# peterarmstrong/corda

Measured on AMD Instinct MI355X. Metric: verified sigs/sec (whole node), Ed25519 + ECDSA-P256, at 1/2/4/8 MI355X, higher is better.
Workload: dtype u32

## Files before the change

corda_amd/csrc/cordagpu.cpp:

```cpp
#include <hip/hip_runtime.h>

#include <algorithm>
#include <atomic>
#include <chrono>
#include <cmath>
#include <cstdio>
#include <cstring>
#include <functional>
#include <initializer_list>
#include <memory>
#include <mutex>
#include <string>
#include <thread>
#include <vector>

#include "../../include/cordagpu.h"
#include "call_scope.h"
#include "engine.h"
#include "host_budget.h"
#include "host_pool.h"
#include "pool.h"
#include "rsa.h"
#include "table_budget.h"
#include "txsig_plan.h"

namespace cg24 {
const cgt::EngineVariant& variant();
}
namespace cg22 {
const cgt::EngineVariant& variant();
}

namespace {

thread_local std::string g_err;

int fail(int code, const char* fmt, const char* detail = "") {
  char buf[512];
  snprintf(buf, sizeof buf, fmt, detail);
  g_err = buf;
  return code;
}

int hip_fail(hipError_t e, const char* where) {
  char buf[512];
  snprintf(buf, sizeof buf, "%s: %s", where, hipGetErrorString(e));
  g_err = buf;
  return e == hipErrorOutOfMemory ? CG_ERR_NOMEM : CG_ERR_DEVICE;
}

#define HIP_TRY(expr, where)               \
  do {                                     \
    hipError_t _e = (expr);                \
    if (_e != hipSuccess) return hip_fail(_e, where); \
  } while (0)

bool env_flag(const char* name, bool dflt) {
  const char* v = getenv(name);
  return v ? (dflt ? v[0] != '0' : v[0] == '1') : dflt;
}
uint64_t env_u64(const char* name, uint64_t dflt) {
  const char* v = getenv(name);
  return v ? (uint64_t)strtoull(v, nullptr, 10) : dflt;
}

struct DevBuf {
  void* p = nullptr;
  size_t cap = 0;
  hipError_t ensure(size_t bytes) { return bytes <= cap ? hipSuccess : replace(bytes + bytes / 4 + 256); }
  hipError_t ensure_exact(size_t bytes) { return bytes <= cap ? hipSuccess : replace(bytes); }
  hipError_t replace(size_t want) {
    release();
    const hipError_t e = hipMalloc(&p, want);
    if (e == hipSuccess) cap = want;
    return e;
  }
  void release() {
    if (p) hipFree(p);
    p = nullptr;
    cap = 0;
  }
};

struct Need {
  DevBuf* buf;
  size_t bytes;
};
hipError_t ensure_all(std::initializer_list<Need> needs) {
  bool grow = false;
  for (const Need& n : needs) grow = grow || n.buf->cap < n.bytes;
  if (!grow) return hipSuccess;
  hipError_t e = hipDeviceSynchronize();
  for (const Need& n : needs)
    if (e == hipSuccess) e = n.buf->ensure(n.bytes);
  return e;
}

hipError_t stage(DevBuf& b, const void* src, size_t bytes, hipStream_t s, size_t room = 0) {
  hipError_t e = b.ensure(std::max<size_t>({bytes, room, 1}));
  if (e == hipSuccess && bytes) e = hipMemcpyAsync(b.p, src, bytes, hipMemcpyHostToDevice, s);
  return e;
}
size_t arena_room(uint64_t arena_len) { return ((arena_len + 3) & ~(uint64_t)3) + 16; }

struct HipStreams {
  using Stream = hipStream_t;
  using Event = hipEvent_t;
  using Error = hipError_t;
  static constexpr Error kOk = hipSuccess;
  Error record(Event e, Stream s) { return hipEventRecord(e, s); }
  Error wait(Stream s, Event e) { return hipStreamWaitEvent(s, e, 0); }
  Error sync(Stream s) { return hipStreamSynchronize(s); }
};

}

struct cg_ctx : cg::CallState<HipStreams> {
  int device = 0;
  uint64_t chunk = CG_DEFAULT_CHUNK_ITEMS;
  bool chunk_set = false;
  bool fault = false;
  cg::Fork fork = {{nullptr, nullptr, nullptr}, nullptr, {nullptr, nullptr, nullptr}, nullptr,
                   {nullptr, nullptr, nullptr}, nullptr};
  std::mutex mu;
  DevBuf keyprep, itemws, keys, items, arena, status, aux0, aux1, aux2;
  void* btab = nullptr;
  const cgt::EngineVariant* eng = nullptr;
  uint64_t tab_bytes = 0;
  DevBuf wide;
  bool rsa = false;
  DevBuf rsakeys, rsalist;
  uint32_t wide_max = cg::kKeyWideMax;
  DevBuf kcache;
  uint32_t wide_slots = 0;
  uint32_t wide_slots_max = cg::kKeyWideMax;
  uint32_t kc_bits = 32;
  bool kc_on = true;
  bool kc_dirty = true;
  bool kc_open = false;
  DevBuf txitems, msgs, tmpls, h_txs, h_comps, h_sigs, h_ids, h_txst;
  DevBuf sig12ws;
  DevBuf txvws, txvio;
  DevBuf ftxws;
  DevBuf bfws, bfin, bfio;
  DevBuf signers, signws;
  uint32_t n_signers = 0;
  DevBuf derivews;
  uint32_t derive_force = 0;
  DevBuf ec_signers, signecws;
  uint32_t n_ec_signers = 0;
  DevBuf rsa_signers, signrsaws;
  uint32_t n_rsa_signers = 0;
  hipStream_t copy2 = nullptr;
  cg::CountScratch count_scratch;
  std::unique_ptr<cg::HostPool> hpool;
  uint32_t host_req = 0;
  uint32_t quota = 1;
  bool counted = false;
  std::vector<hipEvent_t> seg;
  hipEvent_t tev[4] = {};
  std::vector<hipEvent_t> segt;
  std::vector<hipEvent_t> segtab;
  hipEvent_t backt[2] = {nullptr, nullptr};
  std::vector<hipEvent_t> fbt;
  std::vector<double> fbh;
  bool htrace = false;
  cg::StageTimer timer;
};

namespace {

std::atomic<unsigned> g_live_ctx{0};

const cgt::EngineVariant* const kVariants[] = {&cg::variant(), &cg24::variant(), &cg22::variant()};
constexpr int kNumVariants = 3;

std::vector<cgb::TableSet> table_sets() {
  std::vector<cgb::TableSet> v;
  for (const cgt::EngineVariant* e : kVariants) v.push_back({e->fixed_base_bits, (uint64_t)e->btab_bytes()});
  return v;
}

struct SharedTables {
  int device;
  int variant;
  void* p;
  unsigned refs;
};
std::mutex g_tab_mu;
std::vector<SharedTables> g_tabs;

hipError_t acquire_tables(int device, hipStream_t s, uint64_t budget, void** out, int* variant) {
  std::lock_guard<std::mutex> g(g_tab_mu);
  const std::vector<cgb::TableSet> sets = table_sets();
  int held = -1;
  for (const SharedTables& t : g_tabs)
    if (t.device == device && (held < 0 || t.variant < held)) held = t.variant;
  size_t free_b = 0, total_b = 0;
  if (hipMemGetInfo(&free_b, &total_b) != hipSuccess) free_b = 0;
  const int pick = cgb::pick_tables(sets.data(), kNumVariants, budget, free_b, held);
  if (pick < 0) return hipErrorInvalidValue;
  for (SharedTables& t : g_tabs)
    if (t.device == device && t.variant == pick) {
      ++t.refs;
      *out = t.p;
      *variant = pick;
      return hipSuccess;
    }
  hipError_t e = hipErrorOutOfMemory;
  for (int v = pick; v < kNumVariants; ++v) {
    if (budget && sets[v].bytes > budget) continue;
    void* p = nullptr;
    e = hipMalloc(&p, sets[v].bytes);
    if (e == hipSuccess) {
      DevBuf scratch;
      e = scratch.ensure(kVariants[v]->btab_scratch_bytes());
      if (e == hipSuccess) e = kVariants[v]->upload_constants();
      if (e == hipSuccess) e = kVariants[v]->init_btab(p, scratch.p, s);
      if (e == hipSuccess) e = hipStreamSynchronize(s);
      scratch.release();
      if (e == hipSuccess) {
        g_tabs.push_back({device, v, p, 1u});
        *out = p;
        *variant = v;
        return hipSuccess;
      }
      hipFree(p);
    }
    (void)hipGetLastError();
    if (e != hipErrorOutOfMemory || budget) break;
  }
  return e;
}

void release_tables(int device, void* p) {
  std::lock_guard<std::mutex> g(g_tab_mu);
  for (size_t i = 0; i < g_tabs.size(); ++i)
    if (g_tabs[i].device == device && g_tabs[i].p == p) {
      if (--g_tabs[i].refs == 0) {
        hipSetDevice(device);
        hipFree(p);
        g_tabs.erase(g_tabs.begin() + (ptrdiff_t)i);
      }
      return;
    }
}

unsigned host_threads_of(cg_ctx* c, uint64_t n) {
  if (n < (1u << 16)) return 1;
  const unsigned nt = cg::host_threads_for(c->host_req, cg::host_threads_env(), c->quota, g_live_ctx.load());
  if (nt <= 1) c->hpool.reset();
  else if (!c->hpool || c->hpool->threads() != nt) c->hpool.reset(new cg::HostPool(nt - 1));
  return nt;
}

void host_par(cg_ctx* c, uint64_t m, const std::function<void(uint64_t)>& fn) {
  if (m > 1 && c->hpool) {
    c->hpool->run(m, fn);
  } else {
    for (uint64_t t = 0; t < m; ++t) fn(t);
  }
}

HipStreams g_hip;
struct Call : cg::CallScope<HipStreams> {
  Call(cg_ctx* c, Form form) : CallScope(g_hip, *c, form) {}
  hipError_t open(void* hip_stream = nullptr) { return CallScope::open((hipStream_t)hip_stream); }
};

int enter(cg_ctx* c, const char* fn) {
  if (c->fault) return fail(CG_ERR_DEVICE, "%s: device fault (injected by cg_pool_inject_fault)", fn);
  HIP_TRY(hipSetDevice(c->device), "hipSetDevice");
  return CG_OK;
}

uint64_t chunk_of(const cg_ctx* c, uint64_t n) { return cg::equal_chunk(c->chunk, n); }

size_t item_half_bytes(const cg_ctx* c, uint64_t ws_items) { return (c->eng->item_ws_bytes(ws_items) + 255) & ~(size_t)255; }
hipError_t ensure_rsa(cg_ctx* c, uint32_t n_keys, uint64_t n_items) {
  if (!c->rsa) return hipSuccess;
  return ensure_all({{&c->rsakeys, cg::rsa_keys_bytes(n_keys)}, {&c->rsalist, cg::rsa_list_bytes(n_items)}});
}
hipError_t rsa_keyprep(cg_ctx* c, const cg::VerifyReq& r, hipStream_t s) {
  if (!c->rsa) return hipSuccess;
  return cg::launch_rsa_keyprep(r, c->rsakeys.p, s);
}
hipError_t rsa_items(cg_ctx* c, const cg::VerifyReq& r, hipStream_t s) {
  if (!c->rsa || r.n_items == 0) return hipSuccess;
  return cg::launch_rsa_items(r, c->rsakeys.p, c->rsalist.p, s);
}

hipError_t ensure_ws(cg_ctx* c, uint32_t n_keys, uint64_t ws_items, uint64_t call_items = 0) {
  {
// ... 698 lines not shown
  std::lock_guard<std::mutex> g(c->mu);
  if (const int rc = enter(c, "cg_sha256_batch_device")) return rc;
  Call call(c, Call::kDevice);
  HIP_TRY(call.open(hip_stream), "hipStreamWaitEvent");
  HIP_TRY(cg::launch_sha256(d_spans, n, d_arena, arena_len, d_digests, call.stream()), "launch_sha256");
  HIP_TRY(call.close(), "hipEventRecord");
  return CG_OK;
}

static int hash_batch(cg_ctx* c, const cg_span* spans, uint64_t n, const uint8_t* arena, uint64_t arena_len,
                      uint8_t* out, int which) {
  if (!c) return fail(CG_ERR_ARG, "hash batch: ctx is NULL");
  if (n && (!spans || !out)) return fail(CG_ERR_ARG, "hash batch: NULL buffer");
  if (n == 0) return CG_OK;
  const size_t dlen = which == 256 ? 32 : 64;
  std::lock_guard<std::mutex> g(c->mu);
  if (const int rc = enter(c, which == 256 ? "cg_sha256_batch" : "cg_sha512_batch")) return rc;
  hipStream_t s = c->stream;
  Call call(c, Call::kHost);
  HIP_TRY(call.open(), "hipStreamWaitEvent");
  HIP_TRY(stage(c->items, spans, sizeof(cg_span) * n, s), "H2D spans");
  HIP_TRY(stage(c->arena, arena, arena_len, s, arena_room(arena_len)), "H2D arena");
  HIP_TRY(c->aux0.ensure(dlen * n), "hipMalloc(digests)");
  HIP_TRY((which == 256 ? cg::launch_sha256 : cg::launch_sha512)((const cg_span*)c->items.p, n, (const uint8_t*)c->arena.p,
                                                                 arena_len, (uint8_t*)c->aux0.p, s), "launch_sha");
  HIP_TRY(hipMemcpyAsync(out, c->aux0.p, dlen * n, hipMemcpyDeviceToHost, s), "D2H digests");
  HIP_TRY(call.close(), "hipEventRecord");
  HIP_TRY(hipStreamSynchronize(s), "hipStreamSynchronize");
  return CG_OK;
}

int cg_sha256_batch(cg_ctx* c, const cg_span* spans, uint64_t n, const uint8_t* arena, uint64_t arena_len,
                    uint8_t* out) {
  return hash_batch(c, spans, n, arena, arena_len, out, 256);
}
int cg_sha512_batch(cg_ctx* c, const cg_span* spans, uint64_t n, const uint8_t* arena, uint64_t arena_len,
                    uint8_t* out) {
  return hash_batch(c, spans, n, arena, arena_len, out, 512);
}

int cg_tx_ids_device(cg_ctx* c, const cg_tx* d_txs, uint64_t n_tx, const cg_component* d_comps, uint64_t n_comps,
                     const uint8_t* d_arena, uint64_t arena_len, uint8_t* d_ids, uint8_t* d_status,
                     void* hip_stream) {
  if (!c) return fail(CG_ERR_ARG, "cg_tx_ids_device: ctx is NULL");
  std::lock_guard<std::mutex> g(c->mu);
  if (const int rc = enter(c, "cg_tx_ids_device")) return rc;
  HIP_TRY(ensure_all({{&c->aux2, cg::tx_ws_bytes(n_comps)}}), "hipMalloc(leaf ws)");
  Call call(c, Call::kDevice);
  HIP_TRY(call.open(hip_stream), "hipStreamWaitEvent");
  HIP_TRY(cg::launch_tx_ids(d_txs, n_tx, d_comps, n_comps, d_arena, arena_len, d_ids, d_status,
                            (uint8_t*)c->aux2.p, call.stream()), "launch_tx_ids");
  HIP_TRY(call.close(), "hipEventRecord");
  return CG_OK;
}

int cg_tx_ids(cg_ctx* c, const cg_tx* txs, uint64_t n_tx, const cg_component* comps, uint64_t n_comps,
              const uint8_t* arena, uint64_t arena_len, uint8_t* ids_out, uint8_t* status_out) {
  if (!c) return fail(CG_ERR_ARG, "cg_tx_ids: ctx is NULL");
  if (n_tx && (!txs || !ids_out || !status_out)) return fail(CG_ERR_ARG, "cg_tx_ids: NULL buffer");
  if (n_tx == 0) return CG_OK;
  std::lock_guard<std::mutex> g(c->mu);
  if (const int rc = enter(c, "cg_tx_ids")) return rc;
  hipStream_t s = c->stream;
  Call call(c, Call::kHost);
  HIP_TRY(call.open(), "hipStreamWaitEvent");
  HIP_TRY(stage(c->keys, txs, sizeof(cg_tx) * n_tx, s), "H2D txs");
  HIP_TRY(stage(c->items, comps, sizeof(cg_component) * n_comps, s), "H2D comps");
  HIP_TRY(stage(c->arena, arena, arena_len, s, arena_room(arena_len)), "H2D arena");
  HIP_TRY(c->aux0.ensure(32 * n_tx), "hipMalloc(ids)");
  HIP_TRY(c->status.ensure(n_tx), "hipMalloc(status)");
  HIP_TRY(c->aux2.ensure(cg::tx_ws_bytes(n_comps)), "hipMalloc(leaf ws)");
  HIP_TRY(cg::launch_tx_ids((const cg_tx*)c->keys.p, n_tx, (const cg_component*)c->items.p, n_comps,
                            (const uint8_t*)c->arena.p, arena_len, (uint8_t*)c->aux0.p, (uint8_t*)c->status.p,
                            (uint8_t*)c->aux2.p, s), "launch_tx_ids");
  HIP_TRY(hipMemcpyAsync(ids_out, c->aux0.p, 32 * n_tx, hipMemcpyDeviceToHost, s), "D2H ids");
  HIP_TRY(hipMemcpyAsync(status_out, c->status.p, n_tx, hipMemcpyDeviceToHost, s), "D2H status");
  HIP_TRY(call.close(), "hipEventRecord");
  HIP_TRY(hipStreamSynchronize(s), "hipStreamSynchronize");
  return CG_OK;
}

int cg_merkle_roots(cg_ctx* c, const uint8_t* leaves, const uint64_t* first, const uint32_t* count, uint64_t n,
                    uint8_t* roots_out, uint8_t* status_out) {
  if (!c) return fail(CG_ERR_ARG, "cg_merkle_roots: ctx is NULL");
  if (n && (!first || !count || !roots_out || !status_out)) return fail(CG_ERR_ARG, "cg_merkle_roots: NULL buffer");
  if (n == 0) return CG_OK;
  uint64_t total = 0, ws = 0;
  std::vector<uint64_t> wsoff(n);
  for (uint64_t j = 0; j < n; ++j) {
    if (first[j] + count[j] > total) total = first[j] + count[j];
    wsoff[j] = ws;
    ws += count[j];
  }
  std::lock_guard<std::mutex> g(c->mu);
  if (const int rc = enter(c, "cg_merkle_roots")) return rc;
  hipStream_t s = c->stream;
  Call call(c, Call::kHost);
  HIP_TRY(call.open(), "hipStreamWaitEvent");
  HIP_TRY(stage(c->arena, leaves, 32 * total, s), "H2D leaves");
  HIP_TRY(stage(c->keys, first, 8 * n, s), "H2D first");
  HIP_TRY(stage(c->items, count, 4 * n, s), "H2D count");
  HIP_TRY(stage(c->aux2, wsoff.data(), 8 * n, s), "H2D wsoff");
  HIP_TRY(c->aux0.ensure(32 * n), "hipMalloc(roots)");
  HIP_TRY(c->status.ensure(n), "hipMalloc(status)");
  HIP_TRY(c->aux1.ensure(32 * (ws ? ws : 1)), "hipMalloc(ws)");
  HIP_TRY(cg::launch_merkle_roots((const uint8_t*)c->arena.p, (const uint64_t*)c->keys.p, (const uint32_t*)c->items.p,
                                  n, (uint8_t*)c->aux0.p, (uint8_t*)c->status.p, (uint8_t*)c->aux1.p,
                                  (const uint64_t*)c->aux2.p, s),
          "launch_merkle_roots");
  HIP_TRY(hipMemcpyAsync(roots_out, c->aux0.p, 32 * n, hipMemcpyDeviceToHost, s), "D2H roots");
  HIP_TRY(hipMemcpyAsync(status_out, c->status.p, n, hipMemcpyDeviceToHost, s), "D2H status");
  HIP_TRY(call.close(), "hipEventRecord");
  HIP_TRY(hipStreamSynchronize(s), "hipStreamSynchronize");
  return CG_OK;
}

static uint64_t tmpl_slot(const cg_signable_tmpl* tmpls, uint32_t n_tmpls) {
  uint64_t maxlen = 0;
  for (uint32_t k = 0; k < n_tmpls; ++k) {
    const uint64_t l = (uint64_t)tmpls[k].prefix_len + 32u + tmpls[k].suffix_len;
    if (l > maxlen) maxlen = l;
  }
  const uint64_t slot = (maxlen + 15) & ~(uint64_t)15;
  return slot ? slot : 16;
}

struct TxnReq {
  const cg_tx* txs;
  uint64_t n_tx;
  const cg_component* comps;
  uint64_t n_comps;
  const cg_key* keys;
  uint32_t n_keys;
  const cg_txsig* sigs;
  uint64_t n_sigs;
  const cg_signable_tmpl* tmpls;
  uint32_t n_tmpls;
  const uint8_t* arena;
  uint64_t arena_len;
  uint32_t mode;
  uint8_t *ids, *tx_status, *sig_status;
};
static int txn_args(const char* fn, const TxnReq& q, bool host) {
  if (q.n_tx && (!q.txs || !q.ids || !q.tx_status)) return fail(CG_ERR_ARG, "%s: NULL tx buffer", fn);
  if (q.n_sigs && (!q.sigs || !q.sig_status)) return fail(CG_ERR_ARG, "%s: NULL sig buffer", fn);
  if (host && q.n_comps && !q.comps) return fail(CG_ERR_ARG, "%s: comps is NULL", fn);
  if (host && q.n_keys && !q.keys) return fail(CG_ERR_ARG, "%s: keys is NULL", fn);
  if (q.n_tmpls && !q.tmpls) return fail(CG_ERR_ARG, "%s: templates is NULL", fn);
  if (host && q.arena_len && !q.arena) return fail(CG_ERR_ARG, "%s: arena is NULL", fn);
  if (q.mode > CG_MODE_ISVALID) return fail(CG_ERR_ARG, "%s: bad mode", fn);
  return CG_OK;
}

static int verify_transactions_locked(cg_ctx* c, const TxnReq& d, hipStream_t s) {
  const uint64_t slot = tmpl_slot(d.tmpls, d.n_tmpls), msgs_len = cg::tx_msgs_head(d.n_tmpls, slot);
  HIP_TRY(ensure_all({{&c->aux2, cg::tx_ws_bytes(d.n_comps)},
                      {&c->txitems, sizeof(cg_item) * (d.n_sigs ? d.n_sigs : 1)},
                      {&c->msgs, msgs_len ? msgs_len : 16},
                      {&c->tmpls, sizeof(cg_signable_tmpl) * (d.n_tmpls ? d.n_tmpls : 1)}}),
          "hipMalloc(transaction workspace)");
  HIP_TRY(ensure_ws(c, d.n_keys, chunk_of(c, d.n_sigs), d.n_sigs), "hipMalloc(workspace)");
  if (d.n_tmpls)
    HIP_TRY(hipMemcpyAsync(c->tmpls.p, d.tmpls, sizeof(cg_signable_tmpl) * d.n_tmpls, hipMemcpyHostToDevice, s),
            "H2D templates");
  HIP_TRY(cg::launch_tx_ids(d.txs, d.n_tx, d.comps, d.n_comps, d.arena, d.arena_len, d.ids, d.tx_status,
                            (uint8_t*)c->aux2.p, s), "launch_tx_ids");
  if (d.n_sigs) {
    HIP_TRY(cg::launch_tx_sig_items(d.sigs, d.n_sigs, (const cg_signable_tmpl*)c->tmpls.p, d.n_tmpls, d.tx_status,
                                    d.n_tx, d.ids, d.arena, d.arena_len, slot, (cg_item*)c->txitems.p,
                                    (uint8_t*)c->msgs.p, s),
            "launch_tx_sig_items");
    const cg::VerifyReq r = {d.keys, d.n_keys, (const cg_item*)c->txitems.p, d.n_sigs, d.arena, d.arena_len, d.mode,
                             d.sig_status, (const uint8_t*)c->msgs.p, msgs_len};
    HIP_TRY(launch_chunked(c, r, cg::equal_bounds(d.n_sigs, chunk_of(c, d.n_sigs)), s, ChunkOpts{}), "launch_verify");
  }
  return CG_OK;
}

int cg_verify_transactions_device(cg_ctx* c, const cg_tx* d_txs, uint64_t n_tx, const cg_component* d_comps,
                                  uint64_t n_comps, const cg_key* d_keys, uint32_t n_keys, const cg_txsig* d_sigs,
                                  uint64_t n_sigs, const cg_signable_tmpl* tmpls, uint32_t n_tmpls,
                                  const uint8_t* d_arena, uint64_t arena_len, uint32_t mode, uint8_t* d_ids,
                                  uint8_t* d_tx_status, uint8_t* d_sig_status, void* hip_stream) {
  if (!c) return fail(CG_ERR_ARG, "cg_verify_transactions_device: ctx is NULL");
  const TxnReq d = {d_txs, n_tx,  d_comps,   n_comps, d_keys, n_keys, d_sigs,      n_sigs,
                    tmpls, n_tmpls, d_arena, arena_len, mode, d_ids,  d_tx_status, d_sig_status};
  if (const int a = txn_args("cg_verify_transactions_device", d, false)) return a;
  std::lock_guard<std::mutex> g(c->mu);
  if (const int rc = enter(c, "cg_verify_transactions_device")) return rc;
  Call call(c, Call::kDevice);
  HIP_TRY(call.open(hip_stream), "hipStreamWaitEvent");
  if (const int rc = verify_transactions_locked(c, d, call.stream())) return rc;
  HIP_TRY(call.close(), "hipEventRecord");
  return CG_OK;
}

static int verify_transactions_host_locked(cg_ctx* c, const TxnReq& h) {
  if (const int rc = enter(c, "cg_verify_transactions")) return rc;
  hipStream_t s = c->stream;
  Call call(c, Call::kHost);
  HIP_TRY(call.open(), "hipStreamWaitEvent");
  HIP_TRY(stage(c->h_txs, h.txs, sizeof(cg_tx) * h.n_tx, s), "H2D txs");
  HIP_TRY(stage(c->h_comps, h.comps, sizeof(cg_component) * h.n_comps, s), "H2D comps");
  HIP_TRY(stage(c->keys, h.keys, sizeof(cg_key) * h.n_keys, s), "H2D keys");
  HIP_TRY(stage(c->h_sigs, h.sigs, sizeof(cg_txsig) * h.n_sigs, s), "H2D sigs");
  HIP_TRY(stage(c->arena, h.arena, h.arena_len, s, arena_room(h.arena_len)), "H2D arena");
  HIP_TRY(c->h_ids.ensure(32 * (h.n_tx ? h.n_tx : 1)), "hipMalloc(ids)");
  HIP_TRY(c->h_txst.ensure(h.n_tx ? h.n_tx : 1), "hipMalloc(tx status)");
  HIP_TRY(c->status.ensure(h.n_sigs ? h.n_sigs : 1), "hipMalloc(sig status)");
  TxnReq d = h;
  d.txs = (const cg_tx*)c->h_txs.p;
  d.comps = (const cg_component*)c->h_comps.p;
  d.keys = (const cg_key*)c->keys.p;
  d.sigs = (const cg_txsig*)c->h_sigs.p;
  d.arena = (const uint8_t*)c->arena.p;
  d.ids = (uint8_t*)c->h_ids.p;
  d.tx_status = (uint8_t*)c->h_txst.p;
  d.sig_status = (uint8_t*)c->status.p;
  if (const int rc = verify_transactions_locked(c, d, s)) return rc;
  if (h.n_tx) {
    HIP_TRY(hipMemcpyAsync(h.ids, d.ids, 32 * h.n_tx, hipMemcpyDeviceToHost, s), "D2H ids");
    HIP_TRY(hipMemcpyAsync(h.tx_status, d.tx_status, h.n_tx, hipMemcpyDeviceToHost, s), "D2H tx status");
  }
  if (h.n_sigs) HIP_TRY(hipMemcpyAsync(h.sig_status, d.sig_status, h.n_sigs, hipMemcpyDeviceToHost, s), "D2H sig status");
  HIP_TRY(call.close(), "hipEventRecord");
  HIP_TRY(hipStreamSynchronize(s), "hipStreamSynchronize");
  return CG_OK;
}

int cg_verify_transactions(cg_ctx* c, const cg_tx* txs, uint64_t n_tx, const cg_component* comps, uint64_t n_comps,
                           const cg_key* keys, uint32_t n_keys, const cg_txsig* sigs, uint64_t n_sigs,
                           const cg_signable_tmpl* tmpls, uint32_t n_tmpls, const uint8_t* arena,
                           uint64_t arena_len, uint32_t mode, uint8_t* ids_out, uint8_t* tx_status_out,
                           uint8_t* sig_status_out) {
  if (!c) return fail(CG_ERR_ARG, "cg_verify_transactions: ctx is NULL");
  const TxnReq h = {txs,   n_tx,    comps, n_comps,   keys, n_keys,  sigs,          n_sigs,
                    tmpls, n_tmpls, arena, arena_len, mode, ids_out, tx_status_out, sig_status_out};
  if (const int a = txn_args("cg_verify_transactions", h, true)) return a;
  for (uint64_t i = 0; i < n_sigs; ++i) sig_status_out[i] = CG_NOT_RUN;
  if (n_tx == 0 && n_sigs == 0) return CG_OK;
  std::lock_guard<std::mutex> g(c->mu);
  return verify_transactions_host_locked(c, h);
}

static hipError_t ensure_txsig_ws(cg_ctx* c, uint64_t n_sigs, uint32_t n_tmpls, uint64_t slot) {
  return ensure_all({{&c->txitems, sizeof(cg_item) * (n_sigs ? n_sigs : 1)},
                     {&c->msgs, cg::tx_msgs_head(n_tmpls, slot)},
                     {&c->tmpls, sizeof(cg_signable_tmpl) * (n_tmpls ? n_tmpls : 1)}});
}

struct TxsigReq {
  const cg_key* keys;
  uint32_t n_keys;
  const uint8_t* ids;
  uint64_t n_ids;
  cg::SigTable sigs;
  uint64_t n_sigs;
  const cg_signable_tmpl* tmpls;
  uint32_t n_tmpls;
  const uint8_t* arena;
  uint64_t arena_len;
  uint32_t mode;
  uint8_t* status;
  const uint8_t* sig_bytes = nullptr;
  uint64_t sig_bytes_off = 0, sig_bytes_len = 0;
};

struct TxsigSched {
  const std::vector<uint64_t>& bounds;
  cg::KeyUses uses;
  const std::function<hipError_t(uint64_t, uint64_t, uint64_t)>* ready = nullptr;
  const std::vector<uint64_t>* chunk_base = nullptr;
  const uint64_t* d_bases = nullptr;
};
static hipError_t launch_txsig(cg_ctx* c, const TxsigReq& d, uint64_t slot, const TxsigSched& p, hipStream_t s) {
  if (d.n_sigs == 0) return hipSuccess;
  hipError_t e = hipSuccess;
  const cg_signable_tmpl* dt = (const cg_signable_tmpl*)c->tmpls.p;
  if (d.n_tmpls) e = hipMemcpyAsync(c->tmpls.p, d.tmpls, sizeof(cg_signable_tmpl) * d.n_tmpls, hipMemcpyHostToDevice, s);
  if (e == hipSuccess)
    e = cg::launch_tx_sig_templates(dt, d.n_tmpls, d.arena, d.arena_len, slot, d.ids, d.n_ids, (uint8_t*)c->msgs.p, s);
  const std::function<hipError_t(uint64_t, uint64_t, uint64_t)> prepare = [&](uint64_t k, uint64_t first,
                                                                               uint64_t cnt) {
    hipError_t r = p.ready ? (*p.ready)(k, first, cnt) : hipSuccess;
    if (r == hipSuccess && d.sigs.packed())
      r = cg::launch_tx_sig12_range((const cg_txsig_packed*)d.sigs.p, first, cnt, d.sig_bytes_off, d.sig_bytes_len,
                                    p.chunk_base ? (*p.chunk_base)[k] : 0, p.d_bases, dt, d.n_tmpls, d.n_ids,
                                    d.arena_len, (cg_item*)c->txitems.p, c->sig12ws.p, s);
    else if (r == hipSuccess)
      r = cg::launch_tx_sig_range((const cg_txsig*)d.sigs.p, first, cnt, dt, d.n_tmpls, nullptr, d.n_ids, d.ids,
                                  d.arena_len, slot, (cg_item*)c->txitems.p, (uint8_t*)c->msgs.p, s);
    return r;
  };
  const cg::VerifyReq r = {d.keys, d.n_keys, (const cg_item*)c->txitems.p, d.n_sigs, d.arena, d.arena_len, d.mode,
                           d.status, (const uint8_t*)c->msgs.p, cg::tx_msgs_head(d.n_tmpls, slot)};
  if (e == hipSuccess) e = launch_chunked(c, r, p.bounds, s, ChunkOpts{&prepare, &p.uses, p.ready != nullptr});
  return e;
}

static double ms_since(std::chrono::steady_clock::time_point t0) {
  return std::chrono::duration<double, std::milli>(std::chrono::steady_clock::now() - t0).count();
}

struct HostTrace {
  cg_ctx* c;
  const std::chrono::steady_clock::time_point t0;
  const bool on;
  std::vector<double> ht;

  double ms() const { return on ? ms_since(t0) : 0; }
  hipError_t begin(uint64_t nch) {
    c->htrace = on;
    if (!on) return hipSuccess;
    hipError_t e = hipSuccess;
    for (int q = 0; q < 2 && e == hipSuccess; ++q)
      if (!c->backt[q]) e = hipEventCreate(&c->backt[q]);
    while (e == hipSuccess && c->fbt.size() < 3 * nch) {
      hipEvent_t ev;
      e = hipEventCreate(&ev);
      if (e == hipSuccess) c->fbt.push_back(ev);
    }
    c->fbh.assign(nch, 0.0);
    ht.assign(3 * nch, 0.0);
    return e;
  }
  void table_staged(uint64_t k, double h0, double h1) {
    if (!on) return;
    ht[3 * k] = h0;
    ht[3 * k + 1] = h1 - h0;
    ht[3 * k + 2] = ms() - h1;
  }
  hipError_t bytes_staged(uint64_t k, hipStream_t cs, double h2, double h3, double table_mb, const Extent& ek) {
    if (!on) return hipSuccess;
    hipError_t e = hipSuccess;
    while (c->segt.size() <= k) {
      hipEvent_t ev;
      if (hipEventCreate(&ev) != hipSuccess) break;
      c->segt.push_back(ev);
    }
    if (c->segt.size() > k) e = hipEventRecord(c->segt[k], cs);
    fprintf(stderr, "[cg host] chunk %llu at %.3f: scan %.3f sigs %.3f (%.1f MB) ids %.3f arena %.3f (%.1f MB) ms\n",
            (unsigned long long)k, ht[3 * k], ht[3 * k + 1], ht[3 * k + 2], table_mb, h3 - h2, ms() - h3,
            ek.empty() ? 0.0 : (ek.hi - ek.lo) / 1e6);
    return e;
  }
  hipError_t front_reached(uint64_t k, hipStream_t s) {
    if (!on || 3 * k >= c->fbt.size()) return hipSuccess;
    c->fbh[k] = ms();
    return hipEventRecord(c->fbt[3 * k], s);
  }
  void report(uint64_t nch, double h_enq) {
    if (!on) return;
    fprintf(stderr, "[cg host] enqueued at %.3f, done at %.3f ms; copies landed (device ms after the call's first event):",
            h_enq, ms());
    for (uint64_t k = 0; k < nch && k < c->segt.size(); ++k) {
      float t = 0;
      hipEventElapsedTime(&t, c->tev[0], c->segt[k]);
      fprintf(stderr, " %.3f", t);
    }
    float t = 0, f0 = 0, tb = 0;
    hipEventElapsedTime(&t, c->tev[0], c->tev[2]);
    hipEventElapsedTime(&f0, c->tev[0], c->backt[0]);
    hipEventElapsedTime(&tb, c->tev[0], c->backt[1]);
    fprintf(stderr, "; chunk 0 front done %.3f, tables built %.3f, verify done %.3f\n", f0, tb, t);
    for (uint64_t k = 0; k < nch && 3 * k + 2 < c->fbt.size(); ++k) {
      float fs = 0, be = 0, bj = 0;
      hipEventElapsedTime(&fs, c->tev[0], c->fbt[3 * k]);
      hipEventElapsedTime(&bj, c->tev[0], c->fbt[3 * k + 2]);
      hipEventElapsedTime(&be, c->tev[0], c->fbt[3 * k + 1]);
      fprintf(stderr, "[cg host] chunk %llu: front enqueued (host) %.3f, front reached (device) %.3f, back's "
              "kernels done %.3f, joins done %.3f\n", (unsigned long long)k, c->fbh[k], fs, bj, be);
    }
  }
};

struct TxsigFeed {
  cg_ctx* c;
  HostTrace& tr;
  const std::vector<uint64_t>& bounds;
  const TxsigReq& h;
  const TxsigReq& d;
  const uint64_t nt;
  const cg::ParFor& par;
  std::vector<Extent> ext_e, ext_i;
  std::vector<uint64_t> cbase;
  cg::Resident have, have_ids, have_sig;
  hipError_t copy_err = hipSuccess;
  uint64_t mid_k = 0;
  const std::function<hipError_t()> mid_hook = [this] { return mid(); };
  const std::function<hipError_t(uint64_t, uint64_t, uint64_t)> before_hook = [this](uint64_t k, uint64_t, uint64_t) {
    return before(k);
  };

  TxsigFeed(cg_ctx* ctx, HostTrace& trace, const std::vector<uint64_t>& b, const TxsigReq& host, const TxsigReq& dev,
            uint64_t threads, const cg::ParFor& pf)
      : c(ctx), tr(trace), bounds(b), h(host), d(dev), nt(threads), par(pf), ext_e(b.size() - 1),
        ext_i(b.size() - 1), cbase(b.size(), 0) {}
  TxsigFeed(const TxsigFeed&) = delete;
  ~TxsigFeed() { c->fork.mid_front = nullptr; }

  hipError_t copy_table(uint64_t k) {
    const uint64_t first = bounds[k], cnt = bounds[k + 1] - bounds[k];
    const double h0 = tr.ms();
    const cg::ChunkScan x = cg::with_records(h.sigs, [&](auto* recs) {
      return cg::scan_chunk(recs, first, first + cnt, h.n_ids, d.arena_len, nt, par);
    });
    ext_e[k] = x.sig;
    ext_i[k] = x.ids;
    if (h.sigs.packed()) {
      cbase[k + 1] = cbase[k] + x.span;
      ext_e[k] = Extent();
      ext_e[k].add(cbase[k], x.span, h.sig_bytes_len);
    }
    const double h1 = tr.ms();
    const hipError_t e = hipMemcpyAsync((uint8_t*)c->h_sigs.p + (size_t)h.sigs.stride * first, h.sigs.from(first).p,
                                        (size_t)h.sigs.stride * cnt, hipMemcpyHostToDevice, c->copy);
    tr.table_staged(k, h0, h1);
    return e;
  }
  hipError_t copy_bytes(uint64_t k) {
    const Extent& ek = ext_e[k];
    uint8_t* dwin = (uint8_t*)c->arena.p;
    const double h2 = tr.ms();
    hipError_t e = copy_missing(have_ids, ext_i[k], h.ids, (uint8_t*)c->h_ids.p, 0, c->copy);
    const double h3 = tr.ms();
    if (e == hipSuccess && h.sigs.packed()) e = copy_missing(have_sig, ek, h.sig_bytes, dwin + d.sig_bytes_off, 0, c->copy);
    else if (e == hipSuccess) e = copy_missing(have, ek, h.arena, dwin, 0, c->copy);
    if (e == hipSuccess) e = hipEventRecord(c->seg[k], c->copy);
    if (e == hipSuccess) e = tr.bytes_staged(k, c->copy, h2, h3, h.sigs.stride * (bounds[k + 1] - bounds[k]) / 1e6, ek);
    return e;
  }
  hipError_t mid() {
    c->fork.mid_front = nullptr;
    const uint64_t k = mid_k;
// ... 602 lines not shown
  if (!c) return fail(CG_ERR_ARG, "%s: ctx is NULL", fn);
  const cg::BuildOut o{out_base, d_ftxs, d_nodes, node_cap, d_leaves_out, leaf_cap, d_out, out_cap, d_status, d_totals};
  if (!d_totals) return fail(CG_ERR_ARG, "%s: NULL buffer", fn);
  if (const int rc = build_out_args(fn, n, o, true)) return rc;
  if (n && (!d_first || !d_count || !d_inc_first || !d_inc_count || (n_leaf_hashes && !d_leaves) ||
            (n_inc_hashes && !d_include)))
    return fail(CG_ERR_ARG, "%s: NULL buffer", fn);
  if ((((uintptr_t)d_leaves | (uintptr_t)d_include) & 3) != 0)
    return fail(CG_ERR_ARG, "%s: a hash table is not 4-byte aligned", fn);
  const cg::BuildPtIn in{d_leaves, n_leaf_hashes, d_first, d_count, n, leaf_total, d_include, n_inc_hashes,
                         d_inc_first, d_inc_count};
  std::lock_guard<std::mutex> g(c->mu);
  if (const int rc = enter(c, fn)) return rc;
  HIP_TRY(ensure_all({{&c->bfws, cg::build_pt_ws_bytes(n, leaf_total)}}), "hipMalloc(build ws)");
  Call call(c, Call::kDevice);
  HIP_TRY(call.open(hip_stream), "hipStreamWaitEvent");
  HIP_TRY(cg::launch_build_pt_count(in, o, (uint8_t*)c->bfws.p, call.stream()), "launch_build_pt_count");
  HIP_TRY(cg::launch_build_pt_emit(in, o, (uint8_t*)c->bfws.p, call.stream()), "launch_build_pt_emit");
  HIP_TRY(call.close(), "hipEventRecord");
  return CG_OK;
}

int cg_build_partial_trees(cg_ctx* c, const uint8_t* leaves, const uint64_t* first, const uint32_t* count, uint64_t n,
                           const uint8_t* include, const uint64_t* inc_first, const uint32_t* inc_count,
                           uint64_t out_base, cg_filtered_tx* ftxs_out, cg_pmt_node* nodes_out, uint64_t node_cap,
                           cg_filtered_leaf* leaves_out, uint64_t leaf_cap, uint8_t* out, uint64_t out_cap,
                           uint8_t* status_out, cg_build_totals* totals_out) {
  const char* fn = "cg_build_partial_trees";
  if (!c) return fail(CG_ERR_ARG, "%s: ctx is NULL", fn);
  cg::BuildOut h{out_base, ftxs_out, nodes_out, node_cap, leaves_out, leaf_cap, out, out_cap, status_out, totals_out};
  if (!totals_out) return fail(CG_ERR_ARG, "%s: NULL buffer", fn);
  if (const int rc = build_out_args(fn, n, h, false)) return rc;
  if (n && (!first || !count || !inc_first || !inc_count)) return fail(CG_ERR_ARG, "%s: NULL buffer", fn);
  memset(totals_out, 0, sizeof *totals_out);
  if (n == 0) return CG_OK;
  uint64_t n_leaf_hashes = 0, n_inc_hashes = 0, leaf_total = 0;
  for (uint64_t j = 0; j < n; ++j) {
    if (first[j] + count[j] > n_leaf_hashes) n_leaf_hashes = first[j] + count[j];
    if (inc_first[j] + inc_count[j] > n_inc_hashes) n_inc_hashes = inc_first[j] + inc_count[j];
    leaf_total += count[j];
  }
  if ((n_leaf_hashes && !leaves) || (n_inc_hashes && !include)) return fail(CG_ERR_ARG, "%s: NULL buffer", fn);
  std::lock_guard<std::mutex> g(c->mu);
  if (const int rc = enter(c, fn)) return rc;
  hipStream_t s = c->stream;
  Call call(c, Call::kHost);
  HIP_TRY(call.open(), "hipStreamWaitEvent");
  HIP_TRY(stage(c->arena, leaves, 32 * n_leaf_hashes, s), "H2D leaves");
  HIP_TRY(stage(c->aux0, include, 32 * n_inc_hashes, s), "H2D include");
  HIP_TRY(stage(c->keys, first, 8 * n, s), "H2D first");
  HIP_TRY(stage(c->items, count, 4 * n, s), "H2D count");
  HIP_TRY(stage(c->aux1, inc_first, 8 * n, s), "H2D inc_first");
  HIP_TRY(stage(c->aux2, inc_count, 4 * n, s), "H2D inc_count");
  HIP_TRY(c->bfin.ensure(build_fixed_bytes(n)), "hipMalloc(build results)");
  HIP_TRY(c->bfws.ensure(cg::build_pt_ws_bytes(n, leaf_total)), "hipMalloc(build ws)");
  const cg::BuildPtIn in{(const uint8_t*)c->arena.p, n_leaf_hashes, (const uint64_t*)c->keys.p,
                         (const uint32_t*)c->items.p, n, leaf_total, (const uint8_t*)c->aux0.p, n_inc_hashes,
                         (const uint64_t*)c->aux1.p, (const uint32_t*)c->aux2.p};
  cg::BuildOut d = h;
  d.nodes = nullptr;
  d.leaves = nullptr;
  d.out = nullptr;
  build_fixed_split((uint8_t*)c->bfin.p, n, &d);
  HIP_TRY(cg::launch_build_pt_count(in, d, (uint8_t*)c->bfws.p, s), "launch_build_pt_count");
  if (const int rc = build_host_tables(c, fn, h, &d, s)) return rc;
  HIP_TRY(cg::launch_build_pt_emit(in, d, (uint8_t*)c->bfws.p, s), "launch_build_pt_emit");
  if (const int rc = build_host_results(h, d, n, s)) return rc;
  HIP_TRY(call.close(), "hipEventRecord");
  HIP_TRY(hipStreamSynchronize(s), "hipStreamSynchronize");
  return CG_OK;
}

static_assert(sizeof(cg_sign_req) == 8 && sizeof(cg_sign_item) == 16, "sign request layouts");

static int signers_load_locked(cg_ctx* c, const uint8_t* seeds, uint32_t n, uint8_t* pubkeys_out) {
  if (const int rc = enter(c, "cg_signers_load")) return rc;
  signers_drop(c);
  const size_t keys_b = (c->eng->signer_bytes() * n + 255) & ~(size_t)255, seeds_b = 32 * (size_t)n;
  HIP_TRY(c->signers.ensure_exact(keys_b + 2 * seeds_b), "hipMalloc(signers)");
  uint8_t* base = (uint8_t*)c->signers.p;
  uint8_t *d_seeds = base + keys_b, *d_pub = d_seeds + seeds_b;
  hipStream_t s = c->stream;
  hipError_t e;
  {
    Call call(c, Call::kHost);
    e = call.open();
    if (e == hipSuccess) e = hipMemcpyAsync(d_seeds, seeds, seeds_b, hipMemcpyHostToDevice, s);
    if (e == hipSuccess) e = c->eng->launch_signer_expand(d_seeds, n, base, d_pub, c->btab, s);
    if (e == hipSuccess) e = hipMemsetAsync(d_seeds, 0, seeds_b, s);
    if (e == hipSuccess) e = hipMemcpyAsync(pubkeys_out, d_pub, seeds_b, hipMemcpyDeviceToHost, s);
    if (e == hipSuccess) e = call.close();
    if (e == hipSuccess) e = hipStreamSynchronize(s);
  }
  if (e != hipSuccess) {
    signers_drop(c);
    return hip_fail(e, "cg_signers_load");
  }
  c->n_signers = n;
  return CG_OK;
}

int cg_signers_load(cg_ctx* c, const uint8_t* seeds, uint32_t n, uint8_t* pubkeys_out) {
  if (!c) return fail(CG_ERR_ARG, "cg_signers_load: ctx is NULL");
  if (n == 0 || n > CG_SIGNERS_MAX) return fail(CG_ERR_ARG, "cg_signers_load: 1 .. CG_SIGNERS_MAX signers");
  if (!seeds || !pubkeys_out) return fail(CG_ERR_ARG, "cg_signers_load: NULL buffer");
  std::lock_guard<std::mutex> g(c->mu);
  return signers_load_locked(c, seeds, n, pubkeys_out);
}

int cg_signers_clear(cg_ctx* c) {
  if (!c) return fail(CG_ERR_ARG, "cg_signers_clear: ctx is NULL");
  std::lock_guard<std::mutex> g(c->mu);
  HIP_TRY(hipSetDevice(c->device), "hipSetDevice");
  signers_drop(c);
  return CG_OK;
}

struct SignReq {
  const void* reqs;
  uint64_t n;
  bool fused;
  const uint8_t* ids;
  uint64_t n_ids;
  const cg_signable_tmpl* tmpls;
  uint32_t n_tmpls;
  const uint8_t* arena;
  uint64_t arena_len;
  uint8_t* sigs;
  uint8_t* status;
  size_t req_bytes() const { return fused ? sizeof(cg_sign_req) : sizeof(cg_sign_item); }
};

static int sign_args(const char* fn, cg_ctx* c, const SignReq& q, bool host) {
  if (!c) return fail(CG_ERR_ARG, "%s: ctx is NULL", fn);
  if (q.n && (!q.reqs || !q.sigs || !q.status)) return fail(CG_ERR_ARG, "%s: NULL request / signature / status buffer", fn);
  if (q.n_ids && !q.ids) return fail(CG_ERR_ARG, "%s: ids is NULL", fn);
  if (q.n_tmpls && !q.tmpls) return fail(CG_ERR_ARG, "%s: templates is NULL", fn);
  if (q.n_tmpls > 0x10000u) return fail(CG_ERR_ARG, "%s: more than 65536 templates (cg_sign_req.tmpl is 16-bit)", fn);
  if (host && q.arena_len && !q.arena) return fail(CG_ERR_ARG, "%s: arena is NULL", fn);
  return CG_OK;
}

static hipError_t ensure_sign_ws(cg_ctx* c, const SignReq& q, uint64_t slot) {
  return ensure_all({{&c->signws, c->eng->sign_ws_bytes(chunk_of(c, q.n))},
                     {&c->msgs, q.fused ? cg::tx_msgs_head(q.n_tmpls, slot) : 1},
                     {&c->tmpls, sizeof(cg_signable_tmpl) * (q.n_tmpls ? q.n_tmpls : 1)}});
}

static hipError_t launch_sign_call(cg_ctx* c, const SignReq& d, uint64_t slot, hipStream_t s) {
  hipError_t e = hipSuccess;
  const cg_signable_tmpl* dt = (const cg_signable_tmpl*)c->tmpls.p;
  if (d.fused) {
    if (d.n_tmpls) e = hipMemcpyAsync(c->tmpls.p, d.tmpls, sizeof(cg_signable_tmpl) * d.n_tmpls, hipMemcpyHostToDevice, s);
    if (e == hipSuccess)
      e = cg::launch_tx_sig_templates(dt, d.n_tmpls, d.arena, d.arena_len, slot, d.ids, d.n_ids, (uint8_t*)c->msgs.p, s);
  }
  const std::vector<uint64_t> bounds = cg::equal_bounds(d.n, chunk_of(c, d.n));
  for (size_t k = 0; e == hipSuccess && k + 1 < bounds.size(); ++k) {
    const uint64_t first = bounds[k], cnt = bounds[k + 1] - first;
    const cg::SignArgs a = {(const uint8_t*)d.reqs + first * d.req_bytes(), cnt, d.fused, c->signers.p, c->n_signers,
                            d.arena, d.arena_len, (const uint8_t*)c->msgs.p, dt, d.n_tmpls, d.n_ids,
                            d.sigs + 64 * first, d.status + first, c->signws.p, c->btab};
    e = c->eng->launch_sign(a, s);
  }
  const hipError_t z = hipMemsetAsync(c->signws.p, 0, c->eng->sign_ws_bytes(chunk_of(c, d.n)), s);
  return e != hipSuccess ? e : z;
}

static int sign_device(const char* fn, cg_ctx* c, const SignReq& d, void* hip_stream) {
  if (const int a = sign_args(fn, c, d, false)) return a;
  if (d.n == 0) return CG_OK;
  std::lock_guard<std::mutex> g(c->mu);
  if (const int rc = enter(c, fn)) return rc;
  if (c->n_signers == 0) return fail(CG_ERR_ARG, "%s: no signers loaded (cg_signers_load)", fn);
  const uint64_t slot = tmpl_slot(d.tmpls, d.n_tmpls);
  HIP_TRY(ensure_sign_ws(c, d, slot), "hipMalloc(sign workspace)");
  Call call(c, Call::kDevice);
  HIP_TRY(call.open(hip_stream), "hipStreamWaitEvent");
  HIP_TRY(launch_sign_call(c, d, slot, call.stream()), "launch_sign");
  HIP_TRY(call.close(), "hipEventRecord");
  return CG_OK;
}

static int sign_host_locked(const char* fn, cg_ctx* c, const SignReq& h) {
  if (const int rc = enter(c, fn)) return rc;
  if (c->n_signers == 0) return fail(CG_ERR_ARG, "%s: no signers loaded (cg_signers_load)", fn);
  const uint64_t slot = tmpl_slot(h.tmpls, h.n_tmpls);
  HIP_TRY(ensure_sign_ws(c, h, slot), "hipMalloc(sign workspace)");
  hipStream_t s = c->stream;
  Call call(c, Call::kHost);
  HIP_TRY(call.open(), "hipStreamWaitEvent");
  HIP_TRY(stage(c->items, h.reqs, h.req_bytes() * h.n, s), "H2D sign requests");
  HIP_TRY(stage(c->arena, h.arena, h.arena_len, s, arena_room(h.arena_len)), "H2D arena");
  HIP_TRY(stage(c->h_ids, h.ids, 32 * h.n_ids, s), "H2D ids");
  HIP_TRY(c->aux0.ensure(64 * h.n), "hipMalloc(signatures)");
  HIP_TRY(c->status.ensure(h.n), "hipMalloc(status)");
  SignReq d = h;
  d.reqs = c->items.p;
  d.arena = (const uint8_t*)c->arena.p;
  d.ids = (const uint8_t*)c->h_ids.p;
  d.sigs = (uint8_t*)c->aux0.p;
  d.status = (uint8_t*)c->status.p;
  HIP_TRY(launch_sign_call(c, d, slot, s), "launch_sign");
  HIP_TRY(hipMemcpyAsync(h.sigs, d.sigs, 64 * h.n, hipMemcpyDeviceToHost, s), "D2H signatures");
  HIP_TRY(hipMemcpyAsync(h.status, d.status, h.n, hipMemcpyDeviceToHost, s), "D2H status");
  HIP_TRY(call.close(), "hipEventRecord");
  HIP_TRY(hipStreamSynchronize(s), "hipStreamSynchronize");
  return CG_OK;
}

static int sign_host(const char* fn, cg_ctx* c, const SignReq& h) {
  if (const int a = sign_args(fn, c, h, true)) return a;
  if (h.n == 0) return CG_OK;
  std::lock_guard<std::mutex> g(c->mu);
  return sign_host_locked(fn, c, h);
}

int cg_sign_tx_ids(cg_ctx* c, const uint8_t* ids, uint64_t n_ids, const cg_sign_req* reqs, uint64_t n,
                   const cg_signable_tmpl* tmpls, uint32_t n_tmpls, const uint8_t* arena, uint64_t arena_len,
                   uint8_t* sigs_out, uint8_t* status_out) {
  return sign_host("cg_sign_tx_ids", c, {reqs, n, true, ids, n_ids, tmpls, n_tmpls, arena, arena_len, sigs_out, status_out});
}

int cg_sign_tx_ids_device(cg_ctx* c, const uint8_t* d_ids, uint64_t n_ids, const cg_sign_req* d_reqs, uint64_t n,
                          const cg_signable_tmpl* tmpls, uint32_t n_tmpls, const uint8_t* d_arena, uint64_t arena_len,
                          uint8_t* d_sigs, uint8_t* d_status, void* hip_stream) {
  return sign_device("cg_sign_tx_ids_device", c,
                     {d_reqs, n, true, d_ids, n_ids, tmpls, n_tmpls, d_arena, arena_len, d_sigs, d_status}, hip_stream);
}

int cg_sign_batch(cg_ctx* c, const cg_sign_item* items, uint64_t n, const uint8_t* arena, uint64_t arena_len,
                  uint8_t* sigs_out, uint8_t* status_out) {
  return sign_host("cg_sign_batch", c, {items, n, false, nullptr, 0, nullptr, 0, arena, arena_len, sigs_out, status_out});
}

static int ec_signers_load_locked(cg_ctx* c, const uint8_t* schemes, const uint8_t* secrets, uint32_t n,
                                  uint8_t* pubs_out, uint8_t* status_out) {
  if (const int rc = enter(c, "cg_ec_signers_load")) return rc;
  ec_signers_drop(c);
  auto al = [](size_t x) { return (x + 255) & ~(size_t)255; };
  const size_t keys_b = al(c->eng->ec_signer_bytes() * n), d_b = 32 * (size_t)n, pub_b = 64 * (size_t)n;
  HIP_TRY(c->ec_signers.ensure_exact(keys_b + al(d_b) + al(n) + al(pub_b) + al(n)), "hipMalloc(ECDSA signers)");
  uint8_t* base = (uint8_t*)c->ec_signers.p;
  uint8_t *d_d = base + keys_b, *d_sch = d_d + al(d_b), *d_pub = d_sch + al(n), *d_st = d_pub + al(pub_b);
  hipStream_t s = c->stream;
  hipError_t e;
  {
    Call call(c, Call::kHost);
    e = call.open();
    if (e == hipSuccess) e = hipMemcpyAsync(d_d, secrets, d_b, hipMemcpyHostToDevice, s);
    if (e == hipSuccess) e = hipMemcpyAsync(d_sch, schemes, n, hipMemcpyHostToDevice, s);
    if (e == hipSuccess) e = c->eng->launch_ec_signer_expand(d_sch, d_d, n, base, d_pub, d_st, c->btab, s);
    if (e == hipSuccess) e = hipMemsetAsync(d_d, 0, d_b, s);
    if (e == hipSuccess) e = hipMemcpyAsync(pubs_out, d_pub, pub_b, hipMemcpyDeviceToHost, s);
    if (e == hipSuccess) e = hipMemcpyAsync(status_out, d_st, n, hipMemcpyDeviceToHost, s);
    if (e == hipSuccess) e = call.close();
    if (e == hipSuccess) e = hipStreamSynchronize(s);
  }
  if (e != hipSuccess) {
    ec_signers_drop(c);
    return hip_fail(e, "cg_ec_signers_load");
  }
  c->n_ec_signers = n;
  return CG_OK;
}

static int ec_signers_load_args(const char* fn, const uint8_t* schemes, const uint8_t* secrets, uint32_t n,
                                const uint8_t* pubs_out, const uint8_t* status_out) {
  if (n == 0 || n > CG_SIGNERS_MAX) return fail(CG_ERR_ARG, "%s: 1 .. CG_SIGNERS_MAX signers", fn);
  if (!schemes || !secrets || !pubs_out || !status_out) return fail(CG_ERR_ARG, "%s: NULL buffer", fn);
  return CG_OK;
}

int cg_ec_signers_load(cg_ctx* c, const uint8_t* schemes, const uint8_t* secrets, uint32_t n, uint8_t* pubs_out,
                       uint8_t* status_out) {
  if (!c) return fail(CG_ERR_ARG, "cg_ec_signers_load: ctx is NULL");
  if (const int a = ec_signers_load_args("cg_ec_signers_load", schemes, secrets, n, pubs_out, status_out)) return a;
  std::lock_guard<std::mutex> g(c->mu);
  return ec_signers_load_locked(c, schemes, secrets, n, pubs_out, status_out);
}

int cg_ec_signers_clear(cg_ctx* c) {
  if (!c) return fail(CG_ERR_ARG, "cg_ec_signers_clear: ctx is NULL");
  std::lock_guard<std::mutex> g(c->mu);
  HIP_TRY(hipSetDevice(c->device), "hipSetDevice");
  ec_signers_drop(c);
  return CG_OK;
}

struct SignEcReq {
  SignReq q;
  const uint8_t* nonces;
  uint8_t* sig_len;
};

static int sign_ec_args(const char* fn, cg_ctx* c, const SignEcReq& r, bool host) {
  if (const int a = sign_args(fn, c, r.q, host)) return a;
  if (r.q.n && (!r.nonces || !r.sig_len)) return fail(CG_ERR_ARG, "%s: NULL nonce / length buffer", fn);
  return CG_OK;
}

static hipError_t ensure_sign_ec_ws(cg_ctx* c, const SignReq& q, uint64_t slot) {
  return ensure_all({{&c->signecws, c->eng->sign_ec_ws_bytes(chunk_of(c, q.n))},
                     {&c->msgs, q.fused ? cg::tx_msgs_head(q.n_tmpls, slot) : 1},
                     {&c->tmpls, sizeof(cg_signable_tmpl) * (q.n_tmpls ? q.n_tmpls : 1)}});
}

static hipError_t launch_sign_ec_call(cg_ctx* c, const SignEcReq& r, uint64_t slot, hipStream_t s) {
  const SignReq& d = r.q;
  hipError_t e = hipSuccess;
  const cg_signable_tmpl* dt = (const cg_signable_tmpl*)c->tmpls.p;
  if (d.fused) {
    if (d.n_tmpls) e = hipMemcpyAsync(c->tmpls.p, d.tmpls, sizeof(cg_signable_tmpl) * d.n_tmpls, hipMemcpyHostToDevice, s);
    if (e == hipSuccess)
      e = cg::launch_tx_sig_templates(dt, d.n_tmpls, d.arena, d.arena_len, slot, d.ids, d.n_ids, (uint8_t*)c->msgs.p, s);
  }
  const std::vector<uint64_t> bounds = cg::equal_bounds(d.n, chunk_of(c, d.n));
  for (size_t k = 0; e == hipSuccess && k + 1 < bounds.size(); ++k) {
    const uint64_t first = bounds[k], cnt = bounds[k + 1] - first;
    const cg::SignEcArgs a = {(const uint8_t*)d.reqs + first * d.req_bytes(), cnt, d.fused, c->ec_signers.p,
                              c->n_ec_signers, d.arena, d.arena_len, (const uint8_t*)c->msgs.p, dt, d.n_tmpls, d.n_ids,
                              r.nonces + 32 * first, d.sigs + CG_EC_SIG_MAX * first, r.sig_len + first,
                              d.status + first, c->signecws.p, c->btab};
    e = c->eng->launch_sign_ec(a, s);
  }
  const hipError_t z = hipMemsetAsync(c->signecws.p, 0, c->eng->sign_ec_ws_bytes(chunk_of(c, d.n)), s);
  return e != hipSuccess ? e : z;
}

static int sign_ec_device(const char* fn, cg_ctx* c, const SignEcReq& d, void* hip_stream) {
  if (const int a = sign_ec_args(fn, c, d, false)) return a;
  if (d.q.n == 0) return CG_OK;
  std::lock_guard<std::mutex> g(c->mu);
  if (const int rc = enter(c, fn)) return rc;
  if (c->n_ec_signers == 0) return fail(CG_ERR_ARG, "%s: no ECDSA signers loaded (cg_ec_signers_load)", fn);
  const uint64_t slot = tmpl_slot(d.q.tmpls, d.q.n_tmpls);
  HIP_TRY(ensure_sign_ec_ws(c, d.q, slot), "hipMalloc(sign workspace)");
  Call call(c, Call::kDevice);
  HIP_TRY(call.open(hip_stream), "hipStreamWaitEvent");
  HIP_TRY(launch_sign_ec_call(c, d, slot, call.stream()), "launch_sign_ec");
  HIP_TRY(call.close(), "hipEventRecord");
  return CG_OK;
}

static int sign_ec_host_locked(const char* fn, cg_ctx* c, const SignEcReq& h) {
  if (const int rc = enter(c, fn)) return rc;
  if (c->n_ec_signers == 0) return fail(CG_ERR_ARG, "%s: no ECDSA signers loaded (cg_ec_signers_load)", fn);
  const SignReq& q = h.q;
  const uint64_t slot = tmpl_slot(q.tmpls, q.n_tmpls);
  HIP_TRY(ensure_sign_ec_ws(c, q, slot), "hipMalloc(sign workspace)");
  hipStream_t s = c->stream;
  Call call(c, Call::kHost);
  HIP_TRY(call.open(), "hipStreamWaitEvent");
  HIP_TRY(stage(c->items, q.reqs, q.req_bytes() * q.n, s), "H2D sign requests");
  HIP_TRY(stage(c->arena, q.arena, q.arena_len, s, arena_room(q.arena_len)), "H2D arena");
  HIP_TRY(stage(c->h_ids, q.ids, 32 * q.n_ids, s), "H2D ids");
  HIP_TRY(c->aux0.ensure((CG_EC_SIG_MAX + 32 + 1) * q.n), "hipMalloc(signatures)");
  HIP_TRY(c->status.ensure(q.n), "hipMalloc(status)");
  SignEcReq d = h;
  d.q.reqs = c->items.p;
  d.q.arena = (const uint8_t*)c->arena.p;
  d.q.ids = (const uint8_t*)c->h_ids.p;
  d.q.sigs = (uint8_t*)c->aux0.p;
  d.q.status = (uint8_t*)c->status.p;
  uint8_t* d_nonces = d.q.sigs + CG_EC_SIG_MAX * q.n;
  d.nonces = d_nonces;
  d.sig_len = d_nonces + 32 * q.n;
  hipError_t e = hipMemcpyAsync(d_nonces, h.nonces, 32 * q.n, hipMemcpyHostToDevice, s);
  if (e == hipSuccess) e = launch_sign_ec_call(c, d, slot, s);
  const hipError_t z = hipMemsetAsync(d_nonces, 0, 32 * q.n, s);
  if (e == hipSuccess) e = z;
  HIP_TRY(e, "launch_sign_ec");
  HIP_TRY(hipMemcpyAsync(q.sigs, d.q.sigs, CG_EC_SIG_MAX * q.n, hipMemcpyDeviceToHost, s), "D2H signatures");
  HIP_TRY(hipMemcpyAsync(h.sig_len, d.sig_len, q.n, hipMemcpyDeviceToHost, s), "D2H signature lengths");
  HIP_TRY(hipMemcpyAsync(q.status, d.q.status, q.n, hipMemcpyDeviceToHost, s), "D2H status");
  HIP_TRY(call.close(), "hipEventRecord");
  HIP_TRY(hipStreamSynchronize(s), "hipStreamSynchronize");
  return CG_OK;
}

static int sign_ec_host(const char* fn, cg_ctx* c, const SignEcReq& h) {
  if (const int a = sign_ec_args(fn, c, h, true)) return a;
  if (h.q.n == 0) return CG_OK;
  std::lock_guard<std::mutex> g(c->mu);
  return sign_ec_host_locked(fn, c, h);
}

int cg_ec_sign_tx_ids(cg_ctx* c, const uint8_t* ids, uint64_t n_ids, const cg_sign_req* reqs, uint64_t n,
                      const cg_signable_tmpl* tmpls, uint32_t n_tmpls, const uint8_t* arena, uint64_t arena_len,
                      const uint8_t* nonces, uint8_t* sigs_out, uint8_t* sig_len_out, uint8_t* status_out) {
  return sign_ec_host("cg_ec_sign_tx_ids", c,
                      {{reqs, n, true, ids, n_ids, tmpls, n_tmpls, arena, arena_len, sigs_out, status_out}, nonces,
                       sig_len_out});
}

int cg_ec_sign_tx_ids_device(cg_ctx* c, const uint8_t* d_ids, uint64_t n_ids, const cg_sign_req* d_reqs, uint64_t n,
                             const cg_signable_tmpl* tmpls, uint32_t n_tmpls, const uint8_t* d_arena, uint64_t arena_len,
                             const uint8_t* d_nonces, uint8_t* d_sigs, uint8_t* d_sig_len, uint8_t* d_status,
                             void* hip_stream) {
  return sign_ec_device("cg_ec_sign_tx_ids_device", c,
                        {{d_reqs, n, true, d_ids, n_ids, tmpls, n_tmpls, d_arena, arena_len, d_sigs, d_status}, d_nonces,
                         d_sig_len}, hip_stream);
}

int cg_ec_sign_batch(cg_ctx* c, const cg_sign_item* items, uint64_t n, const uint8_t* arena, uint64_t arena_len,
                     const uint8_t* nonces, uint8_t* sigs_out, uint8_t* sig_len_out, uint8_t* status_out) {
  return sign_ec_host("cg_ec_sign_batch", c,
                      {{items, n, false, nullptr, 0, nullptr, 0, arena, arena_len, sigs_out, status_out}, nonces,
                       sig_len_out});
}

static_assert(sizeof(cg_rsa_signer) == 52, "cg_rsa_signer layout");

static int rsa_signers_load_locked(cg_ctx* c, const cg_rsa_signer* signers, uint32_t n, const uint8_t* secrets,
                                   uint64_t secrets_len, uint8_t* status_out) {
  if (const int rc = enter(c, "cg_rsa_signers_load")) return rc;
  rsa_signers_drop(c);
  auto al = [](size_t x) { return (x + 255) & ~(size_t)255; };
  const size_t recs_b = al(cg::rsa_signer_bytes() * n), tab_b = al(sizeof(cg_rsa_signer) * (size_t)n),
               sec_b = al(secrets_len + 4);
  HIP_TRY(c->rsa_signers.ensure_exact(recs_b + tab_b + sec_b + al(n)), "hipMalloc(RSA signers)");
  uint8_t* base = (uint8_t*)c->rsa_signers.p;
  uint8_t *d_tab = base + recs_b, *d_sec = d_tab + tab_b, *d_st = d_sec + sec_b;
  hipStream_t s = c->stream;
  hipError_t e;
  {
    Call call(c, Call::kHost);
    e = call.open();
    if (e == hipSuccess) e = hipMemsetAsync(base, 0, recs_b + tab_b + sec_b + al(n), s);
    if (e == hipSuccess) e = hipMemcpyAsync(d_tab, signers, sizeof(cg_rsa_signer) * (size_t)n, hipMemcpyHostToDevice, s);
    if (e == hipSuccess && secrets_len) e = hipMemcpyAsync(d_sec, secrets, secrets_len, hipMemcpyHostToDevice, s);
    if (e == hipSuccess) e = cg::launch_rsa_signer_expand(d_tab, n, d_sec, secrets_len, base, d_st, s);
    if (e == hipSuccess) e = hipMemsetAsync(d_tab, 0, tab_b + sec_b, s);
    if (e == hipSuccess) e = hipMemcpyAsync(status_out, d_st, n, hipMemcpyDeviceToHost, s);
    if (e == hipSuccess) e = call.close();
    if (e == hipSuccess) e = hipStreamSynchronize(s);
  }
  if (e != hipSuccess) {
    rsa_signers_drop(c);
    return hip_fail(e, "cg_rsa_signers_load");
  }
  c->n_rsa_signers = n;
  return CG_OK;
}

static int rsa_signers_load_args(const char* fn, const cg_rsa_signer* signers, uint32_t n, const uint8_t* secrets,
                                 uint64_t secrets_len, const uint8_t* status_out) {
  if (n == 0 || n > CG_SIGNERS_MAX) return fail(CG_ERR_ARG, "%s: 1 .. CG_SIGNERS_MAX signers", fn);
  if (!signers || !status_out || (secrets_len && !secrets)) return fail(CG_ERR_ARG, "%s: NULL buffer", fn);
  if (secrets_len >= (1ull << 32)) return fail(CG_ERR_ARG, "%s: secrets_len must be below 2^32", fn);
  return CG_OK;
}

int cg_rsa_signers_load(cg_ctx* c, const cg_rsa_signer* signers, uint32_t n, const uint8_t* secrets,
                        uint64_t secrets_len, uint8_t* status_out) {
  if (!c) return fail(CG_ERR_ARG, "cg_rsa_signers_load: ctx is NULL");
  if (const int a = rsa_signers_load_args("cg_rsa_signers_load", signers, n, secrets, secrets_len, status_out)) return a;
  std::lock_guard<std::mutex> g(c->mu);
  return rsa_signers_load_locked(c, signers, n, secrets, secrets_len, status_out);
}

int cg_rsa_signers_clear(cg_ctx* c) {
  if (!c) return fail(CG_ERR_ARG, "cg_rsa_signers_clear: ctx is NULL");
  std::lock_guard<std::mutex> g(c->mu);
  HIP_TRY(hipSetDevice(c->device), "hipSetDevice");
  rsa_signers_drop(c);
  return CG_OK;
}

struct SignRsaReq {
  SignReq q;
  const uint8_t* salts;
  uint16_t* sig_len;
};

static int sign_rsa_args(const char* fn, cg_ctx* c, const SignRsaReq& r, bool host) {
  if (const int a = sign_args(fn, c, r.q, host)) return a;
  if (r.q.n && (!r.salts || !r.sig_len)) return fail(CG_ERR_ARG, "%s: NULL salt / length buffer", fn);
  return CG_OK;
}

static hipError_t ensure_sign_rsa_ws(cg_ctx* c, const SignReq& q, uint64_t slot) {
  return ensure_all({{&c->signrsaws, cg::sign_rsa_ws_bytes(chunk_of(c, q.n))},
                     {&c->msgs, q.fused ? cg::tx_msgs_head(q.n_tmpls, slot) : 1},
                     {&c->tmpls, sizeof(cg_signable_tmpl) * (q.n_tmpls ? q.n_tmpls : 1)}});
}

static hipError_t launch_sign_rsa_call(cg_ctx* c, const SignRsaReq& r, uint64_t slot, hipStream_t s) {
  const SignReq& d = r.q;
  hipError_t e = hipSuccess;
  const cg_signable_tmpl* dt = (const cg_signable_tmpl*)c->tmpls.p;
  if (d.fused) {
    if (d.n_tmpls) e = hipMemcpyAsync(c->tmpls.p, d.tmpls, sizeof(cg_signable_tmpl) * d.n_tmpls, hipMemcpyHostToDevice, s);
    if (e == hipSuccess)
      e = cg::launch_tx_sig_templates(dt, d.n_tmpls, d.arena, d.arena_len, slot, d.ids, d.n_ids, (uint8_t*)c->msgs.p, s);
  }
  const std::vector<uint64_t> bounds = cg::equal_bounds(d.n, chunk_of(c, d.n));
  for (size_t k = 0; e == hipSuccess && k + 1 < bounds.size(); ++k) {
    const uint64_t first = bounds[k], cnt = bounds[k + 1] - first;
    const cg::SignRsaArgs a = {(const uint8_t*)d.reqs + first * d.req_bytes(), cnt, d.fused, c->rsa_signers.p,
                               c->n_rsa_signers, d.arena, d.arena_len, (const uint8_t*)c->msgs.p, dt, d.n_tmpls, d.n_ids,
                               r.salts + 32 * first, d.sigs + CG_RSA_SIG_MAX * first, r.sig_len + first,
                               d.status + first, c->signrsaws.p};
    e = cg::launch_sign_rsa(a, s);
  }
  const hipError_t z = hipMemsetAsync(c->signrsaws.p, 0, cg::sign_rsa_ws_bytes(chunk_of(c, d.n)), s);
  return e != hipSuccess ? e : z;
}

static int sign_rsa_device(const char* fn, cg_ctx* c, const SignRsaReq& d, void* hip_stream) {
  if (const int a = sign_rsa_args(fn, c, d, false)) return a;
  if (d.q.n == 0) return CG_OK;
  std::lock_guard<std::mutex> g(c->mu);
  if (const int rc = enter(c, fn)) return rc;
  if (c->n_rsa_signers == 0) return fail(CG_ERR_ARG, "%s: no RSA signers loaded (cg_rsa_signers_load)", fn);
  const uint64_t slot = tmpl_slot(d.q.tmpls, d.q.n_tmpls);
  HIP_TRY(ensure_sign_rsa_ws(c, d.q, slot), "hipMalloc(sign workspace)");
  Call call(c, Call::kDevice);
  HIP_TRY(call.open(hip_stream), "hipStreamWaitEvent");
  HIP_TRY(launch_sign_rsa_call(c, d, slot, call.stream()), "launch_sign_rsa");
  HIP_TRY(call.close(), "hipEventRecord");
  return CG_OK;
}

static int sign_rsa_host_locked(const char* fn, cg_ctx* c, const SignRsaReq& h) {
  if (const int rc = enter(c, fn)) return rc;
  if (c->n_rsa_signers == 0) return fail(CG_ERR_ARG, "%s: no RSA signers loaded (cg_rsa_signers_load)", fn);
  const SignReq& q = h.q;
  const uint64_t slot = tmpl_slot(q.tmpls, q.n_tmpls);
  HIP_TRY(ensure_sign_rsa_ws(c, q, slot), "hipMalloc(sign workspace)");
  hipStream_t s = c->stream;
  Call call(c, Call::kHost);
  HIP_TRY(call.open(), "hipStreamWaitEvent");
  HIP_TRY(stage(c->items, q.reqs, q.req_bytes() * q.n, s), "H2D sign requests");
  HIP_TRY(stage(c->arena, q.arena, q.arena_len, s, arena_room(q.arena_len)), "H2D arena");
  HIP_TRY(stage(c->h_ids, q.ids, 32 * q.n_ids, s), "H2D ids");
  HIP_TRY(c->aux0.ensure((CG_RSA_SIG_MAX + 32 + 2) * q.n), "hipMalloc(signatures)");
  HIP_TRY(c->status.ensure(q.n), "hipMalloc(status)");
  SignRsaReq d = h;
  d.q.reqs = c->items.p;
  d.q.arena = (const uint8_t*)c->arena.p;
  d.q.ids = (const uint8_t*)c->h_ids.p;
  d.q.sigs = (uint8_t*)c->aux0.p;
  d.q.status = (uint8_t*)c->status.p;
  uint8_t* d_salts = d.q.sigs + CG_RSA_SIG_MAX * q.n;
  d.salts = d_salts;
  d.sig_len = (uint16_t*)(d_salts + 32 * q.n);
  hipError_t e = hipMemcpyAsync(d_salts, h.salts, 32 * q.n, hipMemcpyHostToDevice, s);
  if (e == hipSuccess) e = launch_sign_rsa_call(c, d, slot, s);
  const hipError_t z = hipMemsetAsync(d_salts, 0, 32 * q.n, s);
  if (e == hipSuccess) e = z;
  HIP_TRY(e, "launch_sign_rsa");
  HIP_TRY(hipMemcpyAsync(q.sigs, d.q.sigs, CG_RSA_SIG_MAX * q.n, hipMemcpyDeviceToHost, s), "D2H signatures");
  HIP_TRY(hipMemcpyAsync(h.sig_len, d.sig_len, 2 * q.n, hipMemcpyDeviceToHost, s), "D2H signature lengths");
  HIP_TRY(hipMemcpyAsync(q.status, d.q.status, q.n, hipMemcpyDeviceToHost, s), "D2H status");
  HIP_TRY(call.close(), "hipEventRecord");
  HIP_TRY(hipStreamSynchronize(s), "hipStreamSynchronize");
  return CG_OK;
}

static int sign_rsa_host(const char* fn, cg_ctx* c, const SignRsaReq& h) {
  if (const int a = sign_rsa_args(fn, c, h, true)) return a;
  if (h.q.n == 0) return CG_OK;
  std::lock_guard<std::mutex> g(c->mu);
  return sign_rsa_host_locked(fn, c, h);
}

int cg_rsa_sign_tx_ids(cg_ctx* c, const uint8_t* ids, uint64_t n_ids, const cg_sign_req* reqs, uint64_t n,
                       const cg_signable_tmpl* tmpls, uint32_t n_tmpls, const uint8_t* arena, uint64_t arena_len,
                       const uint8_t* salts, uint8_t* sigs_out, uint16_t* sig_len_out, uint8_t* status_out) {
  return sign_rsa_host("cg_rsa_sign_tx_ids", c,
                       {{reqs, n, true, ids, n_ids, tmpls, n_tmpls, arena, arena_len, sigs_out, status_out}, salts,
                        sig_len_out});
}

int cg_rsa_sign_tx_ids_device(cg_ctx* c, const uint8_t* d_ids, uint64_t n_ids, const cg_sign_req* d_reqs, uint64_t n,
                              const cg_signable_tmpl* tmpls, uint32_t n_tmpls, const uint8_t* d_arena, uint64_t arena_len,
                              const uint8_t* d_salts, uint8_t* d_sigs, uint16_t* d_sig_len, uint8_t* d_status,
                              void* hip_stream) {
  return sign_rsa_device("cg_rsa_sign_tx_ids_device", c,
                         {{d_reqs, n, true, d_ids, n_ids, tmpls, n_tmpls, d_arena, arena_len, d_sigs, d_status}, d_salts,
                          d_sig_len}, hip_stream);
}

int cg_rsa_sign_batch(cg_ctx* c, const cg_sign_item* items, uint64_t n, const uint8_t* arena, uint64_t arena_len,
                      const uint8_t* salts, uint8_t* sigs_out, uint16_t* sig_len_out, uint8_t* status_out) {
  return sign_rsa_host("cg_rsa_sign_batch", c,
                       {{items, n, false, nullptr, 0, nullptr, 0, arena, arena_len, sigs_out, status_out}, salts,
                        sig_len_out});
}

static_assert(sizeof(cg_derive_parent) == 16 && sizeof(cg_derive_req) == 16, "derive request layouts");

struct DeriveReq {
  const cg_derive_parent* parents;
  uint32_t n_parents;
  const cg_derive_req* reqs;
  uint64_t n;
  const uint8_t* arena;
  uint64_t arena_len;
  uint8_t scheme;
  uint8_t* secrets;
  uint8_t* pubs;
  uint8_t* status;
  uint8_t* retries;
  bool derives() const { return reqs != nullptr; }
};

static int derive_args(const char* fn, cg_ctx* c, const DeriveReq& q, bool derives, bool host) {
  if (!c) return fail(CG_ERR_ARG, "%s: ctx is NULL", fn);
  if (q.n && (!q.secrets || !q.pubs || !q.status)) return fail(CG_ERR_ARG, "%s: NULL secret / public key / status buffer", fn);
  if (derives) {
    if (q.n && !q.reqs) return fail(CG_ERR_ARG, "%s: requests is NULL", fn);
    if (q.n_parents && !q.parents) return fail(CG_ERR_ARG, "%s: parents is NULL", fn);
    if (host && q.arena_len && !q.arena) return fail(CG_ERR_ARG, "%s: arena is NULL", fn);
  } else if (q.scheme != CG_EDDSA_ED25519_SHA512 && q.scheme != CG_ECDSA_SECP256K1_SHA256 &&
             q.scheme != CG_ECDSA_SECP256R1_SHA256) {
    return fail(CG_ERR_ARG, "%s: this scheme has no key derivation (Crypto.deriveKeyPair: UnsupportedOperationException)", fn);
  }
  return CG_OK;
}

static hipError_t launch_derive_call(cg_ctx* c, const DeriveReq& d, hipStream_t s) {
  const uint64_t per = chunk_of(c, d.n);
  cg::DeriveArgs a = {d.parents, d.n_parents, d.reqs,    per,      d.arena,  d.arena_len,   d.scheme,
                      c->derive_force, d.secrets, d.pubs, d.status, d.retries, c->derivews.p, c->btab};
  hipError_t e = d.derives() ? c->eng->launch_derive_parents(a, s) : hipSuccess;
  const std::vector<uint64_t> bounds = cg::equal_bounds(d.n, per);
  for (size_t k = 0; e == hipSuccess && k + 1 < bounds.size(); ++k) {
    const uint64_t first = bounds[k];
    a.n = bounds[k + 1] - first;
    a.d_reqs = d.reqs ? d.reqs + first : nullptr;
    a.d_secrets = d.secrets + 32 * first;
    a.d_pubs = d.pubs + 64 * first;
    a.d_status = d.status + first;
    a.d_retries = d.retries ? d.retries + first : nullptr;
    e = c->eng->launch_derive(a, s);
  }
  const hipError_t z = hipMemsetAsync(c->derivews.p, 0, c->eng->derive_ws_bytes(d.n_parents, per), s);
  return e != hipSuccess ? e : z;
}

static hipError_t ensure_derive_ws(cg_ctx* c, const DeriveReq& q) {
  return ensure_all({{&c->derivews, c->eng->derive_ws_bytes(q.n_parents, chunk_of(c, q.n))}});
}

static int derive_device(const char* fn, cg_ctx* c, const DeriveReq& d, bool derives, void* hip_stream) {
  if (const int a = derive_args(fn, c, d, derives, false)) return a;
// ... 582 lines not shown
```

corda_amd/csrc/engine.h:

```cpp
#pragma once
#include <functional>
#include <stdlib.h>
#include <hip/hip_runtime.h>
#include <stdint.h>

#include <vector>

#include "../../include/cordagpu.h"
#include "launch_schedule.h"

namespace cgt {


struct DeviceConsts;
struct WidePool {
  void* ed = nullptr;
  void* ec = nullptr;
  uint32_t cap_ed = 0, cap_ec = 0;
  uint32_t min_ed = 0, min_ec = 0;
  uint32_t slots = 0;
  void* cache = nullptr;
  uint32_t cache_bits = 32;
  bool cache_dirty = false;
};
// ... 146 lines not shown
  uint16_t* d_sig_len;
  uint8_t* d_status;
  void* d_ws;
};

struct DeriveArgs {
  const cg_derive_parent* d_parents;
  uint32_t n_parents;
  const cg_derive_req* d_reqs;
  uint64_t n;
  const uint8_t* d_arena;
  uint64_t arena_len;
  uint8_t scheme;
  uint32_t force_retries;
  uint8_t* d_secrets;
  uint8_t* d_pubs;
  uint8_t* d_status;
  uint8_t* d_retries;
  void* d_ws;
  const void* d_btab;
};

struct EngineVariant {
  uint32_t fixed_base_bits;
  hipError_t (*upload_constants)();
  size_t (*keyprep_bytes)(uint32_t n_keys);
  size_t (*wide_bytes)(uint32_t n_keys, uint64_t n_items, uint32_t max_slots);
  size_t (*wide_slot_bytes)();
  WidePool (*make_wide_pool)(void* base, uint32_t n_keys, uint64_t n_items, uint32_t max_slots, uint32_t alloc_slots);
  uint32_t (*wide_slots)(uint32_t n_keys, uint64_t n_items, uint32_t max_slots);
  size_t (*key_cache_bytes)(uint32_t slots);
  size_t (*btab_bytes)();
  size_t (*btab_scratch_bytes)();
  hipError_t (*init_btab)(void* d_btab, void* d_scratch, hipStream_t stream);
  size_t (*item_ws_bytes)(uint64_t n_items);
  hipError_t (*launch_keyprep)(const VerifyReq& r, void* d_keyprep, hipStream_t stream, const Fork& fork,
                               const WidePool* wide, const KeyUses* src);
  hipError_t (*launch_key_tables)(const Fork& fork, hipStream_t stream);
  hipError_t (*launch_items)(const ItemArgs& a, hipStream_t stream, const Fork& fork);
  hipError_t (*launch_items_plan)(const ItemArgs& a, hipStream_t stream, const Fork& fork);
  hipError_t (*launch_items_front)(const ItemArgs& a, hipStream_t stream, const Fork& fork, bool planned);
  hipError_t (*launch_items_back)(const ItemArgs& a, hipStream_t stream, const Fork& fork);
  size_t (*signer_bytes)();
  size_t (*sign_ws_bytes)(uint64_t n);
  hipError_t (*launch_signer_expand)(const uint8_t* d_seeds, uint32_t n, void* d_signers, uint8_t* d_pubkeys,
                                     const void* d_btab, hipStream_t stream);
  hipError_t (*launch_sign)(const SignArgs& a, hipStream_t stream);
  size_t (*derive_ws_bytes)(uint32_t n_parents, uint64_t n);
  hipError_t (*launch_derive_parents)(const DeriveArgs& a, hipStream_t stream);
  hipError_t (*launch_derive)(const DeriveArgs& a, hipStream_t stream);
  size_t (*ec_signer_bytes)();
  size_t (*sign_ec_ws_bytes)(uint64_t n);
  hipError_t (*launch_ec_signer_expand)(const uint8_t* d_schemes, const uint8_t* d_secrets, uint32_t n, void* d_signers,
                                        uint8_t* d_pubs, uint8_t* d_status, const void* d_btab, hipStream_t stream);
  hipError_t (*launch_sign_ec)(const SignEcArgs& a, hipStream_t stream);
};

}

namespace cg {

using cgt::DeriveArgs;
using cgt::EngineVariant;
using cgt::Fork;
using cgt::ItemArgs;
using cgt::PendingTabs;
using cgt::SignArgs;
using cgt::SignEcArgs;
using cgt::SignRsaArgs;
using cgt::SigTable;
using cgt::StageTimer;
using cgt::VerifyReq;
using cgt::WidePool;
using cgt::with_records;

const EngineVariant& variant();

hipError_t upload_constants();

size_t keyprep_bytes(uint32_t n_keys);
size_t wide_bytes(uint32_t n_keys, uint64_t n_items, uint32_t max_slots = 8192u);
size_t wide_slot_bytes();
constexpr uint32_t kKeyWideMax = 8192u;
WidePool make_wide_pool(void* base, uint32_t n_keys, uint64_t n_items, uint32_t max_slots = 8192u,
                        uint32_t alloc_slots = 0);
uint32_t wide_slots(uint32_t n_keys, uint64_t n_items, uint32_t max_slots);
size_t key_cache_bytes(uint32_t slots);

size_t btab_bytes();
size_t btab_scratch_bytes();
hipError_t init_btab(void* d_btab, void* d_scratch, hipStream_t stream);
size_t item_ws_bytes(uint64_t n_items);
using cgt::KeyUses;
hipError_t launch_keyprep(const VerifyReq& r, void* d_keyprep, hipStream_t stream, const Fork& fork,
                          const WidePool* wide, const KeyUses* src);
hipError_t launch_key_tables(const Fork& fork, hipStream_t stream);
hipError_t launch_items(const ItemArgs& a, hipStream_t stream, const Fork& fork);
hipError_t launch_items_plan(const ItemArgs& a, hipStream_t stream, const Fork& fork);
hipError_t launch_items_front(const ItemArgs& a, hipStream_t stream, const Fork& fork, bool planned);
hipError_t launch_items_back(const ItemArgs& a, hipStream_t stream, const Fork& fork);

size_t signer_bytes();
size_t sign_ws_bytes(uint64_t n);
hipError_t launch_signer_expand(const uint8_t* d_seeds, uint32_t n, void* d_signers, uint8_t* d_pubkeys,
                                const void* d_btab, hipStream_t stream);
hipError_t launch_sign(const SignArgs& a, hipStream_t stream);

hipError_t derive_upload_constants();
size_t derive_ws_bytes(uint32_t n_parents, uint64_t n);
hipError_t launch_derive_parents(const DeriveArgs& a, hipStream_t stream);
hipError_t launch_derive(const DeriveArgs& a, hipStream_t stream);

hipError_t sign_ec_upload_constants();
size_t ec_signer_bytes();
size_t sign_ec_ws_bytes(uint64_t n);
hipError_t launch_ec_signer_expand(const uint8_t* d_schemes, const uint8_t* d_secrets, uint32_t n, void* d_signers,
                                   uint8_t* d_pubs, uint8_t* d_status, const void* d_btab, hipStream_t stream);
hipError_t launch_sign_ec(const SignEcArgs& a, hipStream_t stream);

constexpr uint64_t kRsaSegment = 1ull << 30;
size_t rsa_keys_bytes(uint32_t n_keys);
size_t rsa_list_bytes(uint64_t n_items);
hipError_t launch_rsa_keyprep(const VerifyReq& r, void* d_rsakeys, hipStream_t stream);
hipError_t launch_rsa_items(const VerifyReq& r, const void* d_rsakeys, void* d_rsalist, hipStream_t stream);

size_t rsa_signer_bytes();
size_t sign_rsa_ws_bytes(uint64_t n);
hipError_t launch_rsa_signer_expand(const void* d_signers_in, uint32_t n, const uint8_t* d_secrets, uint64_t secrets_len,
                                    void* d_store, uint8_t* d_status, hipStream_t stream);
hipError_t launch_sign_rsa(const SignRsaArgs& a, hipStream_t stream);

hipError_t launch_sha256(const cg_span* d_spans, uint64_t n, const uint8_t* d_arena, uint64_t arena_len,
                         uint8_t* d_out, hipStream_t stream);
hipError_t launch_sha512(const cg_span* d_spans, uint64_t n, const uint8_t* d_arena, uint64_t arena_len,
                         uint8_t* d_out, hipStream_t stream);

static inline size_t al256(size_t x) { return (x + 255) & ~(size_t)255; }
size_t tx_ws_bytes(uint64_t n_comps);
uint32_t* tx_ws_map(uint8_t* d_leaf_ws, uint64_t n_comps);
hipError_t launch_tx_leaves(const cg_tx* d_txs, uint64_t n_tx, const cg_component* d_comps, uint64_t n_comps,
                            const uint8_t* d_arena, uint64_t arena_len, uint8_t* d_status, uint8_t* d_leaf_ws,
                            hipStream_t stream);
hipError_t launch_tx_ids(const cg_tx* d_txs, uint64_t n_tx, const cg_component* d_comps, uint64_t n_comps,
                         const uint8_t* d_arena, uint64_t arena_len, uint8_t* d_ids, uint8_t* d_status,
                         uint8_t* d_leaf_ws, hipStream_t stream);

uint64_t tx_msgs_head(uint32_t n_tmpls, uint64_t slot);
hipError_t launch_tx_sig_items(const cg_txsig* d_sigs, uint64_t n_sigs, const cg_signable_tmpl* d_tmpls,
                               uint32_t n_tmpls, const uint8_t* d_tx_status, uint64_t n_tx, const uint8_t* d_ids,
                               const uint8_t* d_arena, uint64_t arena_len, uint64_t slot, cg_item* d_items,
                               uint8_t* d_msgs, hipStream_t stream);
hipError_t launch_tx_sig_templates(const cg_signable_tmpl* d_tmpls, uint32_t n_tmpls, const uint8_t* d_arena,
                                   uint64_t arena_len, uint64_t slot, const uint8_t* d_ids, uint64_t n_ids,
                                   uint8_t* d_msgs, hipStream_t stream);
hipError_t launch_tx_sig_range(const cg_txsig* d_sigs, uint64_t first, uint64_t n, const cg_signable_tmpl* d_tmpls,
                               uint32_t n_tmpls, const uint8_t* d_tx_status, uint64_t n_tx, const uint8_t* d_ids,
                               uint64_t arena_len, uint64_t slot, cg_item* d_items, uint8_t* d_msgs,
                               hipStream_t stream);

size_t tx_sig12_scratch_bytes(uint64_t n);
hipError_t launch_tx_sig12_bases(const cg_txsig_packed* d_sigs, uint64_t first, uint64_t n, uint64_t base,
                                 uint64_t* d_bases, hipStream_t stream);
hipError_t launch_tx_sig12_range(const cg_txsig_packed* d_sigs, uint64_t first, uint64_t n, uint64_t sig_region,
                                 uint64_t sig_bytes_len, uint64_t base, const uint64_t* d_bases,
                                 const cg_signable_tmpl* d_tmpls,
                                 uint32_t n_tmpls, uint64_t n_tx, uint64_t arena_len, cg_item* d_items,
                                 void* d_scratch, hipStream_t stream);

hipError_t launch_merkle_roots(const uint8_t* d_leaves, const uint64_t* d_first, const uint32_t* d_count,
                               uint64_t n, uint8_t* d_roots, uint8_t* d_status, uint8_t* d_ws,
                               const uint64_t* d_wsoff, hipStream_t stream);

size_t ftx_ws_bytes(uint64_t n_leaves);
hipError_t launch_filtered(const cg_filtered_tx* d_ftxs, uint64_t n_ftx, const cg_pmt_node* d_nodes, uint64_t n_nodes,
                           const cg_filtered_leaf* d_leaves, uint64_t n_leaves, const uint8_t* d_arena,
                           uint64_t arena_len, uint8_t* d_status, uint8_t* d_ws, hipStream_t stream);

struct BuildOut {
  uint64_t out_base;
  cg_filtered_tx* ftxs;
  cg_pmt_node* nodes;
  uint64_t node_cap;
  cg_filtered_leaf* leaves;
  uint64_t leaf_cap;
  uint8_t* out;
  uint64_t out_cap;
  uint8_t* status;
  cg_build_totals* totals;
};
struct BuildTxIn {
  const cg_tx* txs;
  uint64_t n_tx;
  const cg_component* comps;
  uint64_t n_comps;
  const uint8_t* arena;
  uint64_t arena_len;
  const uint8_t* visible;
};
struct BuildPtIn {
  const uint8_t* leaves;
  uint64_t n_leaf_hashes;
  const uint64_t* first;
  const uint32_t* count;
  uint64_t n;
  uint64_t leaf_total;
  const uint8_t* include;
  uint64_t n_inc_hashes;
  const uint64_t* inc_first;
  const uint32_t* inc_count;
};
size_t build_ws_bytes(uint64_t n_tx, uint64_t n_comps);
hipError_t launch_build_filtered_count(const BuildTxIn& in, const BuildOut& o, uint8_t* d_leaf_ws, uint8_t* d_ws,
                                       hipStream_t stream);
hipError_t launch_build_filtered_emit(const BuildTxIn& in, const BuildOut& o, uint8_t* d_leaf_ws, uint8_t* d_ws,
                                      hipStream_t stream);
size_t build_pt_ws_bytes(uint64_t n, uint64_t leaf_total);
hipError_t launch_build_pt_count(const BuildPtIn& in, const BuildOut& o, uint8_t* d_ws, hipStream_t stream);
hipError_t launch_build_pt_emit(const BuildPtIn& in, const BuildOut& o, uint8_t* d_ws, hipStream_t stream);


struct TxvSet {
  const uint32_t* key_class = nullptr;
  const cg_tx_check* checks = nullptr;
  uint64_t n_tx = 0;
  const uint32_t* reqs = nullptr;
  uint32_t n_reqs = 0;
  const cg_req_node* nodes = nullptr;
  uint32_t n_nodes = 0;
  cg_tx_verdict* verdicts = nullptr;
  uint8_t* req_status = nullptr;
};
size_t tx_verdicts_ws_bytes(uint64_t n_tx);
hipError_t launch_tx_verdicts(const SigTable& d_sigs, uint64_t n_sigs, const uint8_t* d_status, const cg_key* d_keys,
                              uint32_t n_keys, const TxvSet& d, void* d_ws, hipStream_t stream);

}
```

corda_amd/csrc/key_cache.h:

```cpp
#pragma once
#include <stdint.h>

#if defined(__HIPCC__)
#define KC_HD __host__ __device__ inline
#else
#define KC_HD static inline
#endif

#define KC_KEY_WORDS 24u
#define KC_EMPTY 0u
#define KC_PENDING 1u
#define KC_VALID 2u
#define KC_NONE 0xffffffffu

struct KcKey {
  uint32_t tag;
  uint32_t hash;
  uint32_t bytes[KC_KEY_WORDS];
};
struct KcOwner {
  uint32_t state;
  uint32_t pad;
  KcKey key;
};

KC_HD uint32_t kc_ld4(const uint8_t* arena, uint64_t len_rounded, uint64_t off) {
  const uint64_t a0 = off & ~(uint64_t)3;
  const uint32_t sh = (uint32_t)(off & 3) * 8u;
  const uint32_t w0 = a0 < len_rounded ? *(const uint32_t*)(arena + a0) : 0u;
  if (sh == 0) return w0;
  const uint32_t w1 = (a0 + 4) < len_rounded ? *(const uint32_t*)(arena + a0 + 4) : 0u;
  return (w0 >> sh) | (w1 << (32u - sh));
}

KC_HD void kc_key_load(KcKey& k, uint32_t scheme, uint32_t fmt, uint32_t len, const uint8_t* arena, uint64_t arena_len,
                       uint64_t off) {
  const bool ok = len != 0 && len <= 4u * KC_KEY_WORDS && off <= arena_len && len <= arena_len - off;
  k.tag = ok ? (scheme & 0xffu) | (fmt & 0xffu) << 8 | len << 16 : 0u;
  const uint64_t lr = (arena_len + 3) & ~(uint64_t)3;
  uint32_t h = 0x811c9dc5u ^ k.tag;
  for (uint32_t w = 0; w < KC_KEY_WORDS; ++w) {
    uint32_t v = 0;
    if (ok && 4u * w < len) {
      v = kc_ld4(arena, lr, off + 4u * w);
      if (len - 4u * w < 4u) v &= (1u << (8u * (len - 4u * w))) - 1u;
    }
    k.bytes[w] = v;
    h = (h ^ v) * 0x01000193u;
    h ^= h >> 15;
  }
  k.hash = h;
}

KC_HD bool kc_key_equal(const KcKey& a, const KcKey& b) {
  if (a.tag != b.tag || a.tag == 0u) return false;
  uint32_t d = 0;
  for (uint32_t w = 0; w < KC_KEY_WORDS; ++w) d |= a.bytes[w] ^ b.bytes[w];
  return d == 0;
}

KC_HD uint32_t kc_index_size(uint32_t slots) {
  uint32_t t = 16;
  while (t < 2u * slots) t <<= 1;
  return t;
}
KC_HD uint32_t kc_home(uint32_t hash, uint32_t bits, uint32_t size) {
  const uint32_t m = bits >= 32u ? 0xffffffffu : (1u << bits) - 1u;
  return hash & m & (size - 1u);
}

KC_HD bool kc_begin_slot(KcOwner* owners, uint32_t* live, uint32_t s, bool dirty) {
  if (dirty || owners[s].state != KC_VALID) owners[s].state = KC_EMPTY;
  live[s] = 0;
  return owners[s].state == KC_VALID;
}

KC_HD uint32_t kc_cas(uint32_t* p, uint32_t expect, uint32_t val) {
#if defined(__HIP_DEVICE_COMPILE__)
  return atomicCAS(p, expect, val);
#else
  const uint32_t old = *p;
  if (old == expect) *p = val;
  return old;
#endif
}

KC_HD bool kc_index_insert(uint32_t* index, uint32_t size, uint32_t bits, const KcOwner* owners, uint32_t s) {
  uint32_t b = kc_home(owners[s].key.hash, bits, size);
  for (uint32_t n = 0; n < size; ++n, b = (b + 1u) & (size - 1u))
    if (kc_cas(&index[b], 0u, s + 1u) == 0u) return true;
  return false;
}

KC_HD uint32_t kc_probe(const uint32_t* index, uint32_t size, uint32_t bits, const KcOwner* owners, const KcKey& k) {
  if (k.tag == 0u) return KC_NONE;
  uint32_t b = kc_home(k.hash, bits, size);
  for (uint32_t n = 0; n < size; ++n, b = (b + 1u) & (size - 1u)) {
    const uint32_t e = index[b];
    if (e == 0u) return KC_NONE;
    const KcOwner& o = owners[e - 1u];
    if (o.state == KC_VALID && o.key.hash == k.hash && kc_key_equal(o.key, k)) return e - 1u;
  }
  return KC_NONE;
}

KC_HD void kc_part(uint32_t slots, uint32_t t, uint32_t parts, uint32_t& lo, uint32_t& hi) {
  const uint32_t per = (slots + parts - 1u) / parts;
  lo = t * per < slots ? t * per : slots;
  hi = lo + per < slots ? lo + per : slots;
}
KC_HD void kc_free_count(const KcOwner* owners, const uint32_t* live, uint32_t slots, uint32_t t, uint32_t parts,
                         uint32_t cnt[2]) {
  uint32_t lo, hi;
  kc_part(slots, t, parts, lo, hi);
  cnt[0] = cnt[1] = 0;
  for (uint32_t s = lo; s < hi; ++s)
    if (!live[s]) ++cnt[owners[s].state == KC_VALID ? 1 : 0];
}
KC_HD void kc_free_fill(const KcOwner* owners, const uint32_t* live, uint32_t slots, uint32_t t, uint32_t parts,
                        uint32_t base0, uint32_t base1, uint32_t* freelist) {
  uint32_t lo, hi;
  kc_part(slots, t, parts, lo, hi);
  for (uint32_t s = lo; s < hi; ++s)
    if (!live[s]) freelist[owners[s].state == KC_VALID ? base1++ : base0++] = s;
}

KC_HD uint32_t kc_claim(KcOwner* owners, const uint32_t* freelist, uint32_t nfree, uint32_t r, const KcKey& k,
                        bool* evicted) {
  *evicted = false;
  if (r >= nfree) return KC_NONE;
  const uint32_t s = freelist[r];
  *evicted = owners[s].state == KC_VALID;
  owners[s].state = KC_PENDING;
  owners[s].key = k;
  return s;
}

KC_HD bool kc_commit(KcOwner* owners, uint32_t s, bool decoded) {
  if (owners[s].state != KC_PENDING) return false;
  const bool ok = decoded && owners[s].key.tag != 0u;
  owners[s].state = ok ? KC_VALID : KC_EMPTY;
  return ok;
}
```

corda_amd/csrc/txpipe.hip:

```cpp
#include <hip/hip_runtime.h>

#include "engine.h"
#include "keyws.h"
#include "sha2.h"

namespace cg {

__device__ __forceinline__ bool tmpl_ok(const cg_signable_tmpl& t, uint64_t arena_len) {
  return in_arena(t.prefix_off, t.prefix_len, arena_len) && in_arena(t.suffix_off, t.suffix_len, arena_len);
}

__global__ void __launch_bounds__(256) k_txsig_items(const cg_txsig* __restrict__ sigs, uint64_t first, uint64_t n_sigs,
                                                     const cg_signable_tmpl* __restrict__ tmpls, uint32_t n_tmpls,
                                                     const uint8_t* __restrict__ tx_status, uint64_t n_tx,
                                                     uint64_t arena_len, cg_item* __restrict__ items) {
  const uint64_t j = first + (uint64_t)blockIdx.x * blockDim.x + threadIdx.x;
  if (j >= first + n_sigs) return;
  const cg_txsig s = sigs[j];
  cg_item it;
  it.sig_off = s.sig_off;
  it.sig_len = s.sig_len;
  it.reserved1 = 0;
  bool ok = s.tx_idx < n_tx && s.tmpl < n_tmpls;
  if (ok && tx_status) ok = tx_status[s.tx_idx] == 0;
  cg_signable_tmpl t = {0, 0, 0, 0};
  if (ok) {
    t = tmpls[s.tmpl];
    ok = tmpl_ok(t, arena_len);
  }
  if (ok) {
    it.msg_off = s.tx_idx;
    it.msg_len = t.prefix_len + 32u + t.suffix_len;
    it.key_idx = s.key_idx;
    it.reserved0 = CG_ITEM_MSG_WS | CG_ITEM_TMPL | CG_ITEM_FUSED;
    it.reserved1 = s.tmpl;
  } else {
    it.msg_off = 0;
    it.msg_len = 0;
    it.key_idx = 0xffffffffu;
    it.reserved0 = 0;
  }
  items[j] = it;
}

#define SIG12_BLOCK 256
__device__ __forceinline__ uint32_t sig12_span(uint32_t len) { return (len + 3u) & ~3u; }

__device__ __forceinline__ uint32_t wave_incl_scan(uint32_t v) {
  const int lane = (int)(threadIdx.x & 63);
#pragma unroll
  for (int d = 1; d < 64; d <<= 1) {
    const uint32_t u = __shfl_up(v, d, 64);
    if (lane >= d) v += u;
  }
  return v;
}

__global__ void __launch_bounds__(SIG12_BLOCK) k_sig12_blocksum(const cg_txsig_packed* __restrict__ sigs,
                                                                uint64_t first, uint64_t n, uint64_t* __restrict__ sums) {
  const uint64_t j = (uint64_t)blockIdx.x * SIG12_BLOCK + threadIdx.x;
  uint32_t v = j < n ? sig12_span(sigs[first + j].sig_len) : 0u;
#pragma unroll
  for (int d = 32; d >= 1; d >>= 1) v += __shfl_xor(v, d, 64);
  __shared__ uint32_t part[SIG12_BLOCK / 64];
  if ((threadIdx.x & 63) == 0) part[threadIdx.x >> 6] = v;
  __syncthreads();
  if (threadIdx.x == 0) {
    uint64_t t = 0;
    for (int w = 0; w < SIG12_BLOCK / 64; ++w) t += part[w];
    sums[blockIdx.x] = t;
  }
}

__global__ void __launch_bounds__(1024) k_sig12_scan(uint64_t* __restrict__ sums, uint64_t nb, uint64_t base) {
  __shared__ uint64_t sh[1024];
  const uint32_t t = threadIdx.x;
  const uint64_t per = (nb + 1023) / 1024, lo = t * per, hi = lo + per < nb ? lo + per : nb;
  uint64_t s = 0;
  for (uint64_t i = lo; i < hi; ++i) s += sums[i];
  sh[t] = s;
  __syncthreads();
  for (uint32_t d = 1; d < 1024; d <<= 1) {
    const uint64_t u = t >= d ? sh[t - d] : 0;
    __syncthreads();
    sh[t] += u;
    __syncthreads();
  }
  uint64_t run = base + sh[t] - s;
  for (uint64_t i = lo; i < hi; ++i) {
    const uint64_t x = sums[i];
    sums[i] = run;
    run += x;
  }
}

__global__ void __launch_bounds__(SIG12_BLOCK) k_txsig12_items(const cg_txsig_packed* __restrict__ sigs, uint64_t first,
                                                               uint64_t n_sigs, const uint64_t* __restrict__ bases,
                                                               uint64_t sig_region, uint64_t sig_bytes_len,
                                                               const cg_signable_tmpl* __restrict__ tmpls,
                                                               uint32_t n_tmpls, uint64_t n_tx, uint64_t arena_len,
                                                               cg_item* __restrict__ items) {
  const uint64_t jj = (uint64_t)blockIdx.x * SIG12_BLOCK + threadIdx.x;
  const bool live = jj < n_sigs;
  cg_txsig_packed s = {0, 0, 0, 0};
  if (live) s = sigs[first + jj];
  const uint32_t span = live ? sig12_span(s.sig_len) : 0u;
  const uint32_t incl = wave_incl_scan(span);
  __shared__ uint32_t wtot[SIG12_BLOCK / 64];
  if ((threadIdx.x & 63) == 63) wtot[threadIdx.x >> 6] = incl;
  __syncthreads();
  uint32_t wbase = 0;
  for (uint32_t w = 0; w < (threadIdx.x >> 6); ++w) wbase += wtot[w];
  if (!live) return;
  cg_item it;
  const uint64_t so = bases[blockIdx.x] + (wbase + incl - span);
  it.sig_off = sig_region + so;
  it.sig_len = s.sig_len;
  it.reserved1 = 0;
  bool ok = s.tx_idx < n_tx && s.tmpl < n_tmpls && so <= sig_bytes_len && s.sig_len <= sig_bytes_len - so;
  cg_signable_tmpl t = {0, 0, 0, 0};
  if (ok) {
    t = tmpls[s.tmpl];
    ok = tmpl_ok(t, arena_len);
  }
  if (ok) {
    it.msg_off = s.tx_idx;
    it.msg_len = t.prefix_len + 32u + t.suffix_len;
    it.key_idx = s.key_idx;
    it.reserved0 = CG_ITEM_MSG_WS | CG_ITEM_TMPL | CG_ITEM_FUSED;
    it.reserved1 = s.tmpl;
  } else {
    it.msg_off = 0;
    it.msg_len = 0;
    it.key_idx = 0xffffffffu;
    it.reserved0 = 0;
  }
  items[first + jj] = it;
}

size_t tx_sig12_scratch_bytes(uint64_t n) { return 8 * ((n + SIG12_BLOCK - 1) / SIG12_BLOCK + 1); }

hipError_t launch_tx_sig12_bases(const cg_txsig_packed* d_sigs, uint64_t first, uint64_t n, uint64_t base,
                                 uint64_t* d_bases, hipStream_t stream) {
  if (n == 0) return hipSuccess;
  const uint64_t nb = (n + SIG12_BLOCK - 1) / SIG12_BLOCK;
  hipLaunchKernelGGL(k_sig12_blocksum, dim3((unsigned)nb), dim3(SIG12_BLOCK), 0, stream, d_sigs, first, n, d_bases);
  hipLaunchKernelGGL(k_sig12_scan, dim3(1), dim3(1024), 0, stream, d_bases, nb, base);
  return hipGetLastError();
}

hipError_t launch_tx_sig12_range(const cg_txsig_packed* d_sigs, uint64_t first, uint64_t n, uint64_t sig_region,
                                 uint64_t sig_bytes_len, uint64_t base, const uint64_t* d_bases,
                                 const cg_signable_tmpl* d_tmpls,
                                 uint32_t n_tmpls, uint64_t n_tx, uint64_t arena_len, cg_item* d_items,
                                 void* d_scratch, hipStream_t stream) {
  if (n == 0) return hipSuccess;
  const uint64_t* bases = d_bases ? d_bases + first / SIG12_BLOCK : (const uint64_t*)d_scratch;
  if (d_bases && first % SIG12_BLOCK) return hipErrorInvalidValue;
  if (!d_bases) {
    const hipError_t e = launch_tx_sig12_bases(d_sigs, first, n, base, (uint64_t*)d_scratch, stream);
    if (e != hipSuccess) return e;
  }
  hipLaunchKernelGGL(k_txsig12_items, dim3((unsigned)((n + SIG12_BLOCK - 1) / SIG12_BLOCK)), dim3(SIG12_BLOCK), 0,
                     stream, d_sigs, first, n, bases, sig_region, sig_bytes_len, d_tmpls, n_tmpls, n_tx, arena_len,
                     d_items);
  return hipGetLastError();
}

static __host__ __device__ inline uint64_t tx_img_off(uint32_t n_tmpls) { return tmpl_mid_bytes(n_tmpls); }
uint64_t tx_msgs_head(uint32_t n_tmpls, uint64_t slot) {
  return (tx_img_off(n_tmpls) + (uint64_t)n_tmpls * slot + 255) & ~(uint64_t)255;
}

__global__ void __launch_bounds__(64) k_tmpl_prep(const cg_signable_tmpl* __restrict__ tmpls, uint32_t n_tmpls,
                                                  const uint8_t* __restrict__ arena, uint64_t arena_len,
                                                  uint64_t slot, const uint8_t* __restrict__ ids, uint64_t n_ids,
                                                  uint8_t* __restrict__ msgs) {
  const uint32_t t = blockIdx.x;
  if (t == 0 && threadIdx.x == 0) {
    SpliceHdr h;
    h.ids = (uint64_t)(uintptr_t)ids;
    h.n_ids = n_ids;
    h.img_off = tx_img_off(n_tmpls);
    h.slot = slot;
    h.w512_off = tmpl_w512_off(n_tmpls);
    *(SpliceHdr*)msgs = h;
  }
  if (t >= n_tmpls) return;
  const cg_signable_tmpl tm = tmpls[t];
  const bool ok = tmpl_ok(tm, arena_len);
  const uint64_t lr = round4(arena_len);
  auto byte_at = [&](uint64_t x) -> uint32_t {
    if (!ok) return 0u;
    if (x < tm.prefix_len) return cg_ld_bytes4(arena, lr, tm.prefix_off + x) & 0xffu;
    if (x < tm.prefix_len + 32u) return 0u;
    if (x < (uint64_t)tm.prefix_len + 32u + tm.suffix_len)
      return cg_ld_bytes4(arena, lr, tm.suffix_off + (x - tm.prefix_len - 32u)) & 0xffu;
    return 0u;
  };
  uint32_t* img = (uint32_t*)(msgs + tx_img_off(n_tmpls) + (uint64_t)t * slot);
  for (uint32_t w = threadIdx.x; w < slot / 4; w += 64) {
    uint32_t v = 0;
    for (int q = 0; q < 4; ++q) v |= byte_at(4ull * w + q) << (8 * q);
    img[w] = v;
  }
  const bool ed_mid = ok && tm.prefix_len >= TMPL_ED_MID_MIN_PREFIX;
  if (threadIdx.x == 1) {
    uint64_t* wk = ((TmplW512*)(msgs + tmpl_w512_off(n_tmpls)) + t)->wk;
    uint64_t w[16];
    for (int j = 0; j < 16; ++j) {
      uint64_t v = 0;
      for (int q = 0; q < 8; ++q) v = (v << 8) | (ed_mid ? byte_at(64ull + 8u * j + q) : 0u);
      w[j] = v;
      wk[j] = v + cg_k512(j);
    }
    for (int r = 16; r < 80; r += 16)
      for (int j = 0; j < 16; ++j) wk[r + j] = sha512_sched(w, j) + cg_k512(r + j);
  }
  if (threadIdx.x != 0) return;
  TmplMid r;
  sha256_init(r.state);
  r.blocks = 0;
  r.prefix_len = tm.prefix_len;
  r.ed_mid = ed_mid ? 1u : 0u;
  r.pad = 0;
  if (ok) {
    for (uint32_t b = 0; b < tm.prefix_len / 64; ++b) {
      uint32_t w[16];
      for (int j = 0; j < 16; ++j) {
        uint32_t v = 0;
        for (int q = 0; q < 4; ++q) v = (v << 8) | byte_at(64ull * b + 4u * j + q);
        w[j] = v;
      }
      sha256_compress(r.state, w);
      r.blocks = b + 1;
    }
  }
  ((TmplMid*)(msgs + SPLICE_HDR_BYTES))[t] = r;
}

hipError_t launch_tx_sig_templates(const cg_signable_tmpl* d_tmpls, uint32_t n_tmpls, const uint8_t* d_arena,
                                   uint64_t arena_len, uint64_t slot, const uint8_t* d_ids, uint64_t n_ids,
                                   uint8_t* d_msgs, hipStream_t stream) {
  hipLaunchKernelGGL(k_tmpl_prep, dim3(n_tmpls ? n_tmpls : 1), dim3(64), 0, stream, d_tmpls, n_tmpls, d_arena,
                     arena_len, slot, d_ids, n_ids, d_msgs);
  return hipGetLastError();
}

hipError_t launch_tx_sig_range(const cg_txsig* d_sigs, uint64_t first, uint64_t n, const cg_signable_tmpl* d_tmpls,
                               uint32_t n_tmpls, const uint8_t* d_tx_status, uint64_t n_tx, const uint8_t* d_ids,
                               uint64_t arena_len, uint64_t slot, cg_item* d_items, uint8_t* d_msgs,
                               hipStream_t stream) {
  if (n == 0) return hipSuccess;
  const uint32_t B = 256;
  (void)d_ids;
  (void)slot;
  (void)d_msgs;
  hipLaunchKernelGGL(k_txsig_items, dim3((unsigned)((n + B - 1) / B)), dim3(B), 0, stream, d_sigs, first, n, d_tmpls,
                     n_tmpls, d_tx_status, n_tx, arena_len, d_items);
  return hipGetLastError();
}

hipError_t launch_tx_sig_items(const cg_txsig* d_sigs, uint64_t n_sigs, const cg_signable_tmpl* d_tmpls,
                               uint32_t n_tmpls, const uint8_t* d_tx_status, uint64_t n_tx, const uint8_t* d_ids,
                               const uint8_t* d_arena, uint64_t arena_len, uint64_t slot, cg_item* d_items,
                               uint8_t* d_msgs, hipStream_t stream) {
  if (n_sigs == 0) return hipSuccess;
  hipError_t e = launch_tx_sig_templates(d_tmpls, n_tmpls, d_arena, arena_len, slot, d_ids, n_tx, d_msgs, stream);
  if (e == hipSuccess)
    e = launch_tx_sig_range(d_sigs, 0, n_sigs, d_tmpls, n_tmpls, d_tx_status, n_tx, d_ids, arena_len, slot, d_items,
                            d_msgs, stream);
  return e;
}

}
```

corda_amd/csrc/verify.hip:

```cpp
#include "keyws.h"

namespace cg {

__global__ void k_misc_status(const cg_item* __restrict__ items, uint64_t n_items, const cg_key* __restrict__ keys,
                              uint32_t n_keys, uint8_t* __restrict__ status) {
  const uint64_t i = (uint64_t)blockIdx.x * blockDim.x + threadIdx.x;
  if (i >= n_items) return;
  const uint32_t ki = items[i].key_idx;
  if (ki >= n_keys) {
    status[i] = CG_NOT_RUN;
    return;
  }
  const uint8_t s = keys[ki].scheme;
  if (s != CG_EDDSA_ED25519_SHA512 && s != CG_ECDSA_SECP256R1_SHA256 && s != CG_ECDSA_SECP256K1_SHA256)
    status[i] = CG_UNSUPPORTED;
  else if (s == CG_EDDSA_ED25519_SHA512)
    status[i] = CG_NOT_RUN;
}

__global__ void __launch_bounds__(256) k_key_init(uint32_t n_keys, uint32_t all, uint32_t* __restrict__ uses,
                                                  uint8_t* __restrict__ seen, uint32_t* __restrict__ full_count,
                                                  uint32_t* __restrict__ wide_idx, uint32_t* __restrict__ wide_count) {
  const uint32_t i = blockIdx.x * blockDim.x + threadIdx.x;
  if (i < PLAN_CLASSES) full_count[i] = full_count[ROW0_COUNT_AT + i] = full_count[QUART_COUNT_AT + i] = 0;
  if (i == 0) full_count[SKIP_MISMATCH_AT] = 0;
  if (i < PLAN_CLASSES + 2) wide_count[i] = 0;
  if (i >= n_keys) return;
  uses[i] = all ? KEY_USES_ALL : 0u;
  seen[i] = all ? 1 : 0;
  wide_idx[i] = KEY_NOT_WIDE;
}

__global__ void __launch_bounds__(256) k_key_uses(const cg_item* __restrict__ items, uint64_t n_items,
                                                  uint32_t n_keys, uint32_t* __restrict__ uses,
                                                  uint8_t* __restrict__ seen) {
  const uint64_t i = (uint64_t)blockIdx.x * blockDim.x + threadIdx.x;
  if (i >= n_items) return;
  const uint32_t k = items[i].key_idx;
  if (k >= n_keys) return;
  seen[k] = 1;
  if (((uint32_t)i * 0x9E3779B1u) >> 30 == 0) atomicAdd(&uses[k], KEY_USES_SAMPLE);
}

template <class Sig>
__global__ void __launch_bounds__(256) k_key_uses_txsig(const Sig* __restrict__ sigs, uint64_t n,
                                                        uint32_t n_keys, uint32_t* __restrict__ uses,
                                                        uint8_t* __restrict__ seen) {
  const uint64_t i = (uint64_t)blockIdx.x * blockDim.x + threadIdx.x;
  if (i >= n) return;
  const uint32_t k = sigs[i].key_idx;
  if (k >= n_keys) return;
  seen[k] = 1;
  if (((uint32_t)i * 0x9E3779B1u) >> 30 == 0) atomicAdd(&uses[k], KEY_USES_SAMPLE);
}

__global__ void __launch_bounds__(256) k_key_counts(const uint32_t* __restrict__ counts, uint32_t n_keys,
                                                    uint32_t* __restrict__ uses, uint8_t* __restrict__ seen) {
  const uint32_t i = blockIdx.x * blockDim.x + threadIdx.x;
  if (i >= n_keys) return;
  uses[i] = counts[i];
  seen[i] = counts[i] != 0;
}

__device__ __forceinline__ void list_append(int c, uint32_t i, uint32_t n_keys, uint32_t* __restrict__ list,
                                            uint32_t* __restrict__ count) {
  const uint32_t lane = threadIdx.x & 63u;
#pragma unroll
  for (int k = 0; k < PLAN_CLASSES; ++k) {
    const uint64_t m = __ballot(c == k);
    if (m == 0) continue;
    const int leader = __ffsll((long long)m) - 1;
    uint32_t base = 0;
    if ((int)lane == leader) base = atomicAdd(&count[k], (uint32_t)__popcll(m));
    base = __shfl(base, leader, 64);
    if (c == k) list[(size_t)k * n_keys + base + (uint32_t)__popcll(m & ((1ull << lane) - 1ull))] = i;
  }
}

#define KC_BLOCK 1024
__global__ void __launch_bounds__(KC_BLOCK) k_kc_begin(KeyCache kc) {
  const int pool = blockIdx.x;
  KcOwner* owners = kc.owners[pool];
  uint32_t* index = kc.index[pool];
  if (threadIdx.x < KC_CTRS) kc.ctr[pool * KC_CTRS + threadIdx.x] = 0;
  for (uint32_t b = threadIdx.x; b < kc.size; b += KC_BLOCK) index[b] = 0;
  for (uint32_t s = threadIdx.x; s < kc.slots; s += KC_BLOCK) kc_begin_slot(owners, kc.live[pool], s, kc.dirty);
  __syncthreads();
  for (uint32_t s = threadIdx.x; s < kc.slots; s += KC_BLOCK)
    if (owners[s].state == KC_VALID) kc_index_insert(index, kc.size, kc.bits, owners, s);
}

__device__ __forceinline__ void kc_load_key(KcKey& k, const cg_key& key, const uint8_t* arena, uint64_t arena_len) {
  kc_key_load(k, key.scheme, key.fmt, key.len, arena, arena_len, key.off);
}

__global__ void __launch_bounds__(64) k_key_classify(const cg_key* __restrict__ keys, uint32_t n_keys,
                                                     uint32_t* __restrict__ uses, const uint8_t* __restrict__ seen,
                                                     uint32_t* __restrict__ full, uint32_t* __restrict__ full_count,
                                                     uint32_t* __restrict__ wide_idx, uint32_t* __restrict__ wide,
                                                     uint32_t* __restrict__ wide_count, uint32_t* __restrict__ row0,
                                                     uint32_t* __restrict__ quart, uint32_t cap_ed, uint32_t cap_ec,
                                                     uint32_t min_ed, uint32_t min_ec, uint32_t skip_mask,
                                                     const uint8_t* __restrict__ arena, uint64_t arena_len,
                                                     KeyCache kc) {
  const uint32_t i = blockIdx.x * 64 + threadIdx.x;
  int c = -1, cw = -1, c0 = -1, cq = -1;
  bool is_wide = false;
  uint32_t u = 0;
  if (i < n_keys) {
    u = uses[i];
    if (!seen[i]) u = 0;
    else if (u == 0) u = 1;
    uses[i] = u;
  }
  if (i < n_keys && u >= ED_DIRECT_MAX_USES) {
    const uint8_t s = keys[i].scheme;
    c = s == CG_EDDSA_ED25519_SHA512 ? PLAN_ED
      : s == CG_ECDSA_SECP256R1_SHA256 ? PLAN_R1
      : s == CG_ECDSA_SECP256K1_SHA256 ? PLAN_K1
                                       : -1;
    const int pool = c == PLAN_ED ? 0 : 1;
    if (c >= 0 && u >= (pool == 0 ? min_ed : min_ec) && u != KEY_USES_ALL) {
      const uint32_t cap = pool == 0 ? cap_ed : cap_ec;
      if (cap) {
        const uint32_t slot = atomicAdd(&wide_count[PLAN_CLASSES + pool], 1u);
        if (slot < cap) {
          is_wide = true;
          if (!kc.on()) {
            wide_idx[i] = slot;
            cw = c;
          } else {
            KcKey k;
            kc_load_key(k, keys[i], arena, arena_len);
            const uint32_t hit = kc_probe(kc.index[pool], kc.size, kc.bits, kc.owners[pool], k);
            if (hit != KC_NONE) {
              wide_idx[i] = hit;
              kc.live[pool][hit] = 1;
              atomicAdd(&kc.ctr[pool * KC_CTRS + KC_CTR_HITS], 1u);
            } else {
              cw = c;
            }
          }
          c = -1;
        } else if (kc.on()) {
          atomicAdd(&kc.ctr[pool * KC_CTRS + KC_CTR_FELL_BACK], 1u);
        }
      }
    }
  }
  if (i < n_keys && u >= 1 && !is_wide) {
    const uint8_t s = keys[i].scheme;
    c0 = s == CG_EDDSA_ED25519_SHA512 ? PLAN_ED
       : s == CG_ECDSA_SECP256R1_SHA256 ? PLAN_R1
       : s == CG_ECDSA_SECP256K1_SHA256 ? PLAN_K1
                                        : -1;
    if (u >= KEY_QUARTER_MIN_USES && u < ED_DIRECT_MAX_USES) cq = c0;
  }
  if (skip_mask && (c >= 0 || c0 >= 0)) {
    const int cls = c >= 0 ? c : c0;
    const uint32_t f = cls == PLAN_R1 ? 0u : cls == PLAN_K1 ? 1u : 2u;
    if ((skip_mask >> f) & 1u) atomicOr(&full_count[SKIP_MISMATCH_AT], 1u << f);
  }
  list_append(c, i, n_keys, full, full_count);
  list_append(cw, i, n_keys, wide, wide_count);
  list_append(c0, i, n_keys, row0, full_count + ROW0_COUNT_AT);
  list_append(cq, i, n_keys, quart, full_count + QUART_COUNT_AT);
}

__global__ void __launch_bounds__(KC_BLOCK) k_kc_claim(const cg_key* __restrict__ keys, uint32_t n_keys,
                                                       const uint8_t* __restrict__ arena, uint64_t arena_len,
                                                       uint32_t* __restrict__ wide_idx, uint32_t* __restrict__ wide,
                                                       uint32_t* __restrict__ wide_count, uint32_t* __restrict__ full,
                                                       uint32_t* __restrict__ full_count, uint32_t* __restrict__ row0,
                                                       uint32_t skip_mask, KeyCache kc) {
  __shared__ uint32_t sc[2][KC_BLOCK];
  __shared__ uint32_t tot[2];
  const int pool = blockIdx.x;
  const uint32_t t = threadIdx.x;
  KcOwner* owners = kc.owners[pool];
  uint32_t cnt[2];
  kc_free_count(owners, kc.live[pool], kc.slots, t, KC_BLOCK, cnt);
  sc[0][t] = cnt[0];
  sc[1][t] = cnt[1];
  __syncthreads();
  for (uint32_t d = 1; d < KC_BLOCK; d <<= 1) {
    const uint32_t a = t >= d ? sc[0][t - d] : 0u, b = t >= d ? sc[1][t - d] : 0u;
    __syncthreads();
    sc[0][t] += a;
    sc[1][t] += b;
    __syncthreads();
  }
  if (t == KC_BLOCK - 1) {
    tot[0] = sc[0][t];
    tot[1] = sc[1][t];
  }
  __syncthreads();
  kc_free_fill(owners, kc.live[pool], kc.slots, t, KC_BLOCK, sc[0][t] - cnt[0], tot[0] + sc[1][t] - cnt[1],
               kc.freel[pool]);
  const uint32_t nfree = tot[0] + tot[1];
  const int c_lo = pool == 0 ? PLAN_ED : PLAN_R1, c_hi = pool == 0 ? PLAN_ED : PLAN_K1;
  static_assert(PLAN_R1 + 1 == PLAN_K1, "the ECDSA pool's classes are adjacent");
  uint32_t n_c[2] = {0, 0};
  for (int c = c_lo; c <= c_hi; ++c) n_c[c - c_lo] = wide_count[c];
  __syncthreads();
  uint32_t base = 0;
  for (int c = c_lo; c <= c_hi; ++c) {
    const uint32_t n = n_c[c - c_lo];
    for (uint32_t l = t; l < n; l += KC_BLOCK) {
      const uint32_t i = wide[(size_t)c * n_keys + l];
      KcKey k;
      kc_load_key(k, keys[i], arena, arena_len);
      bool evicted;
      const uint32_t s = kc_claim(owners, kc.freel[pool], nfree, base + l, k, &evicted);
      if (s != KC_NONE) {
        wide_idx[i] = s;
        if (evicted) atomicAdd(&kc.ctr[pool * KC_CTRS + KC_CTR_EVICTED], 1u);
      } else {
        full[(size_t)c * n_keys + atomicAdd(&full_count[c], 1u)] = i;
        row0[(size_t)c * n_keys + atomicAdd(&full_count[ROW0_COUNT_AT + c], 1u)] = i;
        const uint32_t f = c == PLAN_R1 ? 0u : c == PLAN_K1 ? 1u : 2u;
        if ((skip_mask >> f) & 1u) atomicOr(&full_count[SKIP_MISMATCH_AT], 1u << f);
        atomicAdd(&kc.ctr[pool * KC_CTRS + KC_CTR_FELL_BACK], 1u);
      }
    }
    if (t == 0) wide_count[c] = base >= nfree ? 0u : (n < nfree - base ? n : nfree - base);
    base += n;
  }
}

__global__ void __launch_bounds__(256) k_kc_commit(int c, uint32_t n_keys, const EdKeyHdr* __restrict__ hdr,
                                                   const uint32_t* __restrict__ wide,
                                                   const uint32_t* __restrict__ wide_count,
                                                   const uint32_t* __restrict__ wide_idx, KeyCache kc) {
  const int pool = c == PLAN_ED ? 0 : 1;
  const uint32_t n = wide_count[c];
  for (uint32_t l = blockIdx.x * blockDim.x + threadIdx.x; l < n; l += gridDim.x * blockDim.x) {
    const uint32_t i = wide[(size_t)c * n_keys + l];
    if (kc_commit(kc.owners[pool], wide_idx[i], hdr[i].status == 0))
      atomicAdd(&kc.ctr[pool * KC_CTRS + KC_CTR_BUILT], 1u);
  }
}
void kc_launch_commit(int c, uint32_t n_keys, const KeyWs& w, hipStream_t stream) {
  if (!w.kc.on()) return;
  hipLaunchKernelGGL(k_kc_commit, dim3(8), dim3(256), 0, stream, c, n_keys, (const EdKeyHdr*)w.hdr,
                     (const uint32_t*)w.wide, (const uint32_t*)w.wide_count, (const uint32_t*)w.wide_idx, w.kc);
}

__global__ void __launch_bounds__(256) k_mode_guard(const uint32_t* __restrict__ ranges,
                                                    const uint32_t* __restrict__ perm,
                                                    const uint32_t* __restrict__ full_count, uint32_t skip_mask,
                                                    uint8_t* __restrict__ status) {
  const uint32_t bad = full_count[SKIP_MISMATCH_AT] & skip_mask;
  if (!bad) return;
  for (int f = 0; f < 3; ++f) {
    if (!((bad >> f) & 1u)) continue;
    const int cls = f == 0 ? PLAN_R1 : f == 1 ? PLAN_K1 : PLAN_ED;
    const uint32_t beg = ranges[cls], end = ranges[PLAN_WIDE + cls];
    for (uint32_t p = beg + blockIdx.x * blockDim.x + threadIdx.x; p < end; p += gridDim.x * blockDim.x)
      status[perm[p]] = CG_NOT_RUN;
  }
}

hipError_t upload_constants() {
  hipError_t e = ed_upload_constants();
  if (e != hipSuccess) return e;
  e = ec_upload_constants();
  if (e != hipSuccess) return e;
  e = derive_upload_constants();
  if (e != hipSuccess) return e;
  return sign_ec_upload_constants();
}

size_t keyprep_bytes(uint32_t n_keys) { return key_ws_bytes(n_keys); }
size_t wide_bytes(uint32_t n_keys, uint64_t n_items, uint32_t max_slots) {
  return wide_pool_bytes(wide_cap(n_keys, n_items, max_slots));
}
size_t wide_slot_bytes() { return wide_pool_bytes(1); }
static_assert(kKeyWideMax == KEY_WIDE_MAX, "engine.h mirrors keyws.h");
WidePool make_wide_pool(void* base, uint32_t n_keys, uint64_t n_items, uint32_t max_slots, uint32_t alloc_slots) {
  return wide_pool(base, wide_cap(n_keys, n_items, max_slots), alloc_slots);
}
uint32_t wide_slots(uint32_t n_keys, uint64_t n_items, uint32_t max_slots) { return wide_cap(n_keys, n_items, max_slots); }
size_t key_cache_bytes(uint32_t slots) { return key_cache_total(slots); }
size_t item_ws_bytes(uint64_t n_items) { return item_ws_total(n_items); }
size_t btab_bytes() { return const_tab_bytes(); }
size_t btab_scratch_bytes() { return const_scratch_bytes(); }

hipError_t init_btab(void* d_btab, void* d_scratch, hipStream_t stream) {
  hipError_t e = ed_init_const(d_btab, d_scratch, stream);
  if (e != hipSuccess) return e;
  return ec_init_const(d_btab, d_scratch, stream);
}


static void families_needing_full(const KeyUses& src, uint32_t n_keys, const KeyWs& w, bool need[3]) {
  uint32_t hot[2] = {0, 0};
  bool low[3] = {false, false, false};
  for (uint32_t i = 0; i < n_keys; ++i) {
    const uint32_t u = src.host_counts[i];
    if (u == 0) continue;
    const uint8_t s = src.host_keys[i].scheme;
    const int f = s == CG_ECDSA_SECP256R1_SHA256 ? 0 : s == CG_ECDSA_SECP256K1_SHA256 ? 1 : s == CG_EDDSA_ED25519_SHA512 ? 2 : -1;
    if (f < 0) continue;
    const int pool = f == 2 ? 0 : 1;
    const uint32_t cap = pool == 0 ? w.cap_ed : w.cap_ec;
    if (u >= ED_DIRECT_MAX_USES && u >= (pool == 0 ? w.min_ed : w.min_ec) && u != KEY_USES_ALL && cap) ++hot[pool];
    else low[f] = true;
  }
  const bool over[2] = {hot[0] > w.cap_ed, hot[1] > w.cap_ec};
  for (int f = 0; f < 3; ++f) need[f] = low[f] || over[f == 2 ? 0 : 1];
}

struct KeyArgs {
  const VerifyReq& r;
  const cg_item* d_items;
  uint64_t n_items;
  const KeyUses* src;
  KeyWs w;
  uint32_t all;
};

struct HipOps {
  using Error = hipError_t;
  static constexpr Error kOk = hipSuccess;
  hipStream_t main;
  const Fork& fork;
  const KeyArgs* key = nullptr;
  const ItemArgs* a = nullptr;
  KeyWs w{};
  ItemWs iw{};

  HipOps(hipStream_t s, const Fork& f, const KeyArgs* k, const ItemArgs* items) : main(s), fork(f), key(k), a(items) {
    if (!a) return;
    w = key_ws((void*)a->d_keyprep, a->n_keys, a->wide);
    iw = item_ws(a->d_item_ws, a->n_items);
  }
  hipStream_t st(cgs::Stream s) const { return s == cgs::MAIN ? main : fork.side[s - cgs::SIDE0]; }
  hipEvent_t ev(cgs::Event e) const {
    switch (e) {
      case cgs::EV_START: return fork.start;
      case cgs::EV_PLANNED: return fork.planned;
      case cgs::EV_READY0: case cgs::EV_READY1: case cgs::EV_READY2: return fork.ready[e - cgs::EV_READY0];
      case cgs::EV_FRONT: return fork.front;
      case cgs::EV_ROW0_0: case cgs::EV_ROW0_1: case cgs::EV_ROW0_2: return fork.row0[e - cgs::EV_ROW0_0];
      case cgs::EV_EC_FRONT_GO: return fork.ec_front_go;
      case cgs::EV_EC_FRONT_DONE0: case cgs::EV_EC_FRONT_DONE1: return fork.ec_front_done[e - cgs::EV_EC_FRONT_DONE0];
      default: return nullptr;
    }
  }
  Error record(cgs::Event e, cgs::Stream s) { return hipEventRecord(ev(e), st(s)); }
  Error wait(cgs::Stream s, cgs::Event e) { return hipStreamWaitEvent(st(s), ev(e), 0); }
  bool mid_hook() const { return fork.mid_front != nullptr; }
  void before_joins() {
    if (fork.mark) hipEventRecord(fork.mark, main);
  }

  Error run(cgs::Stage stage, cgs::Stream on, int, int) {
    hipStream_t s = st(on);
    switch (stage) {
      case cgs::ST_KEY_INIT: {
        const uint32_t n = key->r.n_keys, kl = n > PLAN_CLASSES + 2 ? n : PLAN_CLASSES + 2;
        hipLaunchKernelGGL(k_key_init, dim3((kl + 255) / 256), dim3(256), 0, s, n, key->all, key->w.uses, key->w.seen,
                           key->w.full_count, key->w.wide_idx, key->w.wide_count);
        return kOk;
      }
      case cgs::ST_KEY_USES:
        hipLaunchKernelGGL(k_key_uses, dim3((unsigned)((key->n_items + 255) / 256)), dim3(256), 0, s, key->d_items,
                           key->n_items, key->r.n_keys, key->w.uses, key->w.seen);
        return kOk;
      case cgs::ST_KEY_COUNTS:
        hipLaunchKernelGGL(k_key_counts, dim3((key->r.n_keys + 255) / 256), dim3(256), 0, s, key->src->counts,
                           key->r.n_keys, key->w.uses, key->w.seen);
        return kOk;
      case cgs::ST_KEY_USES_TXSIG:
        with_records(key->src->sigs, [&](auto* recs) {
          using Rec = std::remove_const_t<std::remove_pointer_t<decltype(recs)>>;
          hipLaunchKernelGGL(k_key_uses_txsig<Rec>, dim3((unsigned)((key->src->n + 255) / 256)), dim3(256), 0, s, recs,
                             key->src->n, key->r.n_keys, key->w.uses, key->w.seen);
        });
        return kOk;
      case cgs::ST_KC_BEGIN:
        hipLaunchKernelGGL(k_kc_begin, dim3(2), dim3(KC_BLOCK), 0, s, key->w.kc);
        return kOk;
      case cgs::ST_KEY_CLASSIFY: {
        const KeyWs& kw = key->w;
        hipLaunchKernelGGL(k_key_classify, dim3((key->r.n_keys + 63) / 64), dim3(64), 0, s, key->r.d_keys, key->r.n_keys,
                           kw.uses, (const uint8_t*)kw.seen, kw.full, kw.full_count, kw.wide_idx, kw.wide, kw.wide_count,
                           kw.row0, kw.quart, kw.cap_ed, kw.cap_ec, kw.min_ed, kw.min_ec, fork.pending.skip_mask,
                           key->r.d_arena, key->r.arena_len, kw.kc);
        return kOk;
      }
      case cgs::ST_KC_CLAIM: {
        const KeyWs& kw = key->w;
        hipLaunchKernelGGL(k_kc_claim, dim3(2), dim3(KC_BLOCK), 0, s, key->r.d_keys, key->r.n_keys, key->r.d_arena,
                           key->r.arena_len, kw.wide_idx, kw.wide, kw.wide_count, kw.full, kw.full_count, kw.row0,
                           fork.pending.skip_mask, kw.kc);
        return kOk;
      }
      case cgs::ST_CHAINS_R1: case cgs::ST_CHAINS_K1:
        ec_launch_keyprep_chains(stage == cgs::ST_CHAINS_R1 ? CG_CURVE_R1 : CG_CURVE_K1, key->r.d_keys, key->r.n_keys,
                                 key->r.d_arena, key->r.arena_len, key->w, s);
        return kOk;
      case cgs::ST_CHAINS_ED:
        ed_launch_keyprep_chains(key->r.d_keys, key->r.n_keys, key->r.d_arena, key->r.arena_len, key->w, s);
        return kOk;
      case cgs::ST_WIDE_TABS_R1: case cgs::ST_WIDE_TABS_K1: case cgs::ST_WIDE_TABS_ED:
      case cgs::ST_FULL_TABS_R1: case cgs::ST_FULL_TABS_K1: case cgs::ST_FULL_TABS_ED: {
        const PendingTabs& p = fork.pending;
        const KeyWs pw = key_ws(p.keyprep, p.n_keys, &p.wide);
        const bool full = stage >= cgs::ST_FULL_TABS_R1;
        const int k = stage - (full ? cgs::ST_FULL_TABS_R1 : cgs::ST_WIDE_TABS_R1);
        if (k == 2) ed_launch_keyprep_tabs(p.keys, p.n_keys, pw, s, full, !full);
        else ec_launch_keyprep_tabs(k == 0 ? CG_CURVE_R1 : CG_CURVE_K1, p.keys, p.n_keys, pw, s, full, !full);
        return kOk;
      }
      case cgs::ST_ED_ABYTE:
        ed_launch_key_abyte(key->r.d_keys, key->r.n_keys, key->r.d_arena, key->r.arena_len, key->w, s);
        return kOk;
      case cgs::ST_MISC_STATUS:
        hipLaunchKernelGGL(k_misc_status, dim3((unsigned)((a->n_items + 255) / 256)), dim3(256), 0, s, a->d_items,
                           a->n_items, a->d_keys, a->n_keys, a->d_status);
        return kOk;
      case cgs::ST_PLAN: {
        Error e = kOk;
        CG_TIME(fork, CG_STAGE_PLAN, s, e = launch_plan(a->d_items, a->n_items, a->d_keys, a->n_keys, w, iw, s));
        return e;
      }
      case cgs::ST_MID_HOOK: return (*fork.mid_front)();
      case cgs::ST_EC_FRONT_R1: case cgs::ST_EC_FRONT_K1: {
        const bool r1 = stage == cgs::ST_EC_FRONT_R1;
        CG_TIME(fork, r1 ? CG_STAGE_R1_FRONT : CG_STAGE_K1_FRONT, s,
                ec_launch_front(r1 ? CG_CURVE_R1 : CG_CURVE_K1, a->d_items, a->n_items, a->d_arena, a->arena_len, a->mode,
                                a->d_status, w, a->d_msgs, a->msgs_len, iw, s));
        return kOk;
      }
      case cgs::ST_ED_FRONT:
        CG_TIME(fork, CG_STAGE_ED_HASH, s,
                ed_launch_front(a->d_items, a->n_items, a->d_arena, a->arena_len, a->mode, a->d_status, w, a->d_msgs,
                                a->msgs_len, iw, s));
        return kOk;
      case cgs::ST_ROW0_LADDER_ED:
        CG_TIME(fork, CG_STAGE_ED_LADDER_ROW0, s,
                ed_launch_ladder(false, a->d_items, a->n_items, a->d_status, w, iw, a->d_btab, s));
        return kOk;
      case cgs::ST_ROW0_LADDER_R1: case cgs::ST_ROW0_LADDER_K1: {
        const bool r1 = stage == cgs::ST_ROW0_LADDER_R1;
        CG_TIME(fork, r1 ? CG_STAGE_R1_LADDER_ROW0 : CG_STAGE_K1_LADDER_ROW0, s,
                ec_launch_ladder(r1 ? CG_CURVE_R1 : CG_CURVE_K1, false, a->d_items, a->n_items, a->d_status, w, iw,
                                 a->d_btab, s));
        return kOk;
      }
      case cgs::ST_FULL_LADDER_ED:
        CG_TIME(fork, CG_STAGE_ED_LADDER, s,
                ed_launch_ladder(true, a->d_items, a->n_items, a->d_status, w, iw, a->d_btab, s));
        return kOk;
      case cgs::ST_WIDE_LADDER_ED:
        CG_TIME(fork, CG_STAGE_ED_LADDER_WIDE, s,
                ed_launch_ladder_wide(a->d_items, a->n_items, a->d_status, w, iw, a->d_btab, s));
        return kOk;
      case cgs::ST_ED_FINISH:
        CG_TIME(fork, CG_STAGE_ED_FINISH, s,
                ed_launch_finish(a->d_items, a->n_items, a->d_arena, a->arena_len, a->d_status, iw, s));
        return kOk;
      case cgs::ST_FULL_LADDER_R1: case cgs::ST_FULL_LADDER_K1: {
        const bool r1 = stage == cgs::ST_FULL_LADDER_R1;
        CG_TIME(fork, r1 ? CG_STAGE_R1_LADDER : CG_STAGE_K1_LADDER, s,
                ec_launch_ladder(r1 ? CG_CURVE_R1 : CG_CURVE_K1, true, a->d_items, a->n_items, a->d_status, w, iw,
                                 a->d_btab, s));
        return kOk;
      }
      case cgs::ST_WIDE_LADDER_R1: case cgs::ST_WIDE_LADDER_K1: {
        const bool r1 = stage == cgs::ST_WIDE_LADDER_R1;
        CG_TIME(fork, r1 ? CG_STAGE_R1_LADDER_WIDE : CG_STAGE_K1_LADDER_WIDE, s,
                ec_launch_ladder_wide(r1 ? CG_CURVE_R1 : CG_CURVE_K1, a->d_items, a->n_items, a->d_status, w, iw,
                                      a->d_btab, s));
        return kOk;
      }
      case cgs::ST_MODE_GUARD:
        hipLaunchKernelGGL(k_mode_guard, dim3(64), dim3(256), 0, s, (const uint32_t*)iw.ranges, (const uint32_t*)iw.perm,
                           (const uint32_t*)w.full_count, fork.pending.skip_mask, a->d_status);
        return kOk;
      default: return hipErrorInvalidValue;
    }
  }
};
using Sched = cgs::Schedule<HipOps>;

static cgs::Chunk chunk_of(const HipOps& ops) {
  cgs::Chunk c;
  c.wide_ed = ops.w.cap_ed != 0;
  c.wide_ec = ops.w.cap_ec != 0;
  return c;
}

hipError_t launch_key_tables(const Fork& fork, hipStream_t stream) {
  HipOps ops(stream, fork, nullptr, nullptr);
  return Sched(ops, fork.pending).key_tables();
}

hipError_t launch_keyprep(const VerifyReq& r, void* d_keyprep, hipStream_t stream, const Fork& fork,
                          const WidePool* wide, const KeyUses* src) {
  const uint32_t n_keys = r.n_keys;
  const cg_item* d_items = src ? nullptr : r.d_items;
  const uint64_t n_items = src ? src->n : r.n_items;
  const bool counted = d_items || src;
  const KeyArgs key = {r, d_items, n_items, src, key_ws(d_keyprep, n_keys, counted ? wide : nullptr), counted ? 0u : 1u};
  cgs::KeyPlan k;
  k.any_keys = n_keys != 0;
  k.counted = counted;
  if (d_items && n_items) k.uses = cgs::ST_KEY_USES;
  else if (src && src->counts) k.uses = cgs::ST_KEY_COUNTS;
  else if (src && src->sigs.p && src->n) k.uses = cgs::ST_KEY_USES_TXSIG;
  if (n_keys && !d_items && src && src->counts && src->host_counts && src->host_keys)
    families_needing_full(*src, n_keys, key.w, k.need_full);
  static const uint32_t test_skip = [] {
    const char* v = getenv("CG_TEST_SKIP_FAMILIES");
    return v ? (uint32_t)strtoul(v, nullptr, 0) & 7u : 0u;
  }();
  for (int f = 0; f < 3; ++f)
    if ((test_skip >> f) & 1u) k.need_full[f] = false;
  k.cache = key.w.kc.on();
  k.wide_ed = key.w.cap_ed != 0;
  k.wide_ec = key.w.cap_ec != 0;
  if (n_keys) {
    fork.pending.keys = r.d_keys;
    fork.pending.n_keys = n_keys;
    fork.pending.keyprep = d_keyprep;
    fork.pending.wide = counted && wide ? *wide : WidePool{};
  }
  HipOps ops(stream, fork, &key, nullptr);
  const hipError_t e = Sched(ops, fork.pending).keyprep(k);
  return e != hipSuccess || n_keys == 0 ? e : hipGetLastError();
}

hipError_t launch_items_plan(const ItemArgs& a, hipStream_t stream, const Fork& fork) {
  if (a.n_items == 0) return hipSuccess;
  HipOps ops(stream, fork, nullptr, &a);
  return Sched(ops, fork.pending).items_plan(chunk_of(ops));
}

hipError_t launch_items_front(const ItemArgs& a, hipStream_t stream, const Fork& fork, bool planned) {
  if (a.n_items == 0) return hipSuccess;
  HipOps ops(stream, fork, nullptr, &a);
  const hipError_t e = Sched(ops, fork.pending).items_front(chunk_of(ops), planned);
  return e != hipSuccess ? e : hipGetLastError();
}

hipError_t launch_items_back(const ItemArgs& a, hipStream_t stream, const Fork& fork) {
  if (a.n_items == 0) return hipSuccess;
  HipOps ops(stream, fork, nullptr, &a);
  const hipError_t e = Sched(ops, fork.pending).items_back(chunk_of(ops));
  return e != hipSuccess ? e : hipGetLastError();
}

hipError_t launch_items(const ItemArgs& a, hipStream_t stream, const Fork& fork) {
  const hipError_t e = launch_items_front(a, stream, fork, false);
  return e != hipSuccess ? e : launch_items_back(a, stream, fork);
}

static_assert(ED_WIDE_BW == EC_WIDE_GW, "one fixed-base radix per build (Makefile VARIANTS)");
const EngineVariant& variant() {
  static const EngineVariant v = {(uint32_t)ED_WIDE_BW, upload_constants, keyprep_bytes, wide_bytes, wide_slot_bytes,
                                  make_wide_pool, wide_slots, key_cache_bytes, btab_bytes, btab_scratch_bytes, init_btab, item_ws_bytes,
                                  launch_keyprep, launch_key_tables, launch_items, launch_items_plan,
                                  launch_items_front, launch_items_back,
                                  signer_bytes, sign_ws_bytes, launch_signer_expand, launch_sign,
                                  derive_ws_bytes, launch_derive_parents, launch_derive,
                                  ec_signer_bytes, sign_ec_ws_bytes, launch_ec_signer_expand, launch_sign_ec};
  return v;
}

}
```

Baseline: 448.8 million.

## Keep template prefixes across calls, parallelize sig12 scan, and use LDS key-use histograms

Several unrelated changes land together. Template message prep can now skip rewriting message heads when the buffer, template count and slot are unchanged since the last call. The single-block sig12 prefix scan becomes a multi-tile, wave-shuffle scan writing to a separate output. Key-use counting gains an LDS histogram kernel with sampled counts, key classification aggregates atomics per wave through ballots, and kc_begin and key hashing batch their loads. Together these aim to cut redundant prep work, serial scan latency and atomic contention. The costs are more complex cache-validity tracking and approximate sampled use counts.

```diff
diff --git a/corda_amd/csrc/cordagpu.cpp b/corda_amd/csrc/cordagpu.cpp
--- a/corda_amd/csrc/cordagpu.cpp
+++ b/corda_amd/csrc/cordagpu.cpp
@@ -67,6 +67,7 @@
 struct DevBuf {
   void* p = nullptr;
   size_t cap = 0;
+  uint64_t allocs = 0;
   hipError_t ensure(size_t bytes) { return bytes <= cap ? hipSuccess : replace(bytes + bytes / 4 + 256); }
   hipError_t ensure_exact(size_t bytes) { return bytes <= cap ? hipSuccess : replace(bytes); }
   hipError_t replace(size_t want) {
@@ -79,6 +80,7 @@
     if (p) hipFree(p);
     p = nullptr;
     cap = 0;
+    ++allocs;
   }
 };
 
@@ -139,6 +141,12 @@
   bool kc_dirty = true;
   bool kc_open = false;
   DevBuf txitems, msgs, tmpls, h_txs, h_comps, h_sigs, h_ids, h_txst;
+  struct {
+    bool valid = false;
+    uint64_t allocs = 0;
+    uint32_t n_tmpls = 0;
+    uint64_t slot = 0;
+  } tmpl_kept;
   DevBuf sig12ws;
   DevBuf txvws, txvio;
   DevBuf ftxws;
@@ -1143,6 +1151,19 @@
   return CG_OK;
 }
 
+static hipError_t launch_templates(cg_ctx* c, uint32_t n_tmpls, const uint8_t* d_arena, uint64_t arena_len,
+                                   uint64_t slot, const uint8_t* d_ids, uint64_t n_ids, hipStream_t s) {
+  auto& k = c->tmpl_kept;
+  const bool keep = k.valid && k.allocs == c->msgs.allocs && k.n_tmpls == n_tmpls && k.slot == slot;
+  const hipError_t e = cg::launch_tx_sig_templates((const cg_signable_tmpl*)c->tmpls.p, n_tmpls, d_arena, arena_len,
+                                                   slot, d_ids, n_ids, (uint8_t*)c->msgs.p, s, keep);
+  k.valid = e == hipSuccess;
+  k.allocs = c->msgs.allocs;
+  k.n_tmpls = n_tmpls;
+  k.slot = slot;
+  return e;
+}
+
 static int verify_transactions_locked(cg_ctx* c, const TxnReq& d, hipStream_t s) {
   const uint64_t slot = tmpl_slot(d.tmpls, d.n_tmpls), msgs_len = cg::tx_msgs_head(d.n_tmpls, slot);
   HIP_TRY(ensure_all({{&c->aux2, cg::tx_ws_bytes(d.n_comps)},
@@ -1157,6 +1178,7 @@
   HIP_TRY(cg::launch_tx_ids(d.txs, d.n_tx, d.comps, d.n_comps, d.arena, d.arena_len, d.ids, d.tx_status,
                             (uint8_t*)c->aux2.p, s), "launch_tx_ids");
   if (d.n_sigs) {
+    c->tmpl_kept.valid = false;
     HIP_TRY(cg::launch_tx_sig_items(d.sigs, d.n_sigs, (const cg_signable_tmpl*)c->tmpls.p, d.n_tmpls, d.tx_status,
                                     d.n_tx, d.ids, d.arena, d.arena_len, slot, (cg_item*)c->txitems.p,
                                     (uint8_t*)c->msgs.p, s),
@@ -1269,8 +1291,7 @@
   hipError_t e = hipSuccess;
   const cg_signable_tmpl* dt = (const cg_signable_tmpl*)c->tmpls.p;
   if (d.n_tmpls) e = hipMemcpyAsync(c->tmpls.p, d.tmpls, sizeof(cg_signable_tmpl) * d.n_tmpls, hipMemcpyHostToDevice, s);
-  if (e == hipSuccess)
-    e = cg::launch_tx_sig_templates(dt, d.n_tmpls, d.arena, d.arena_len, slot, d.ids, d.n_ids, (uint8_t*)c->msgs.p, s);
+  if (e == hipSuccess) e = launch_templates(c, d.n_tmpls, d.arena, d.arena_len, slot, d.ids, d.n_ids, s);
   const std::function<hipError_t(uint64_t, uint64_t, uint64_t)> prepare = [&](uint64_t k, uint64_t first,
                                                                                uint64_t cnt) {
     hipError_t r = p.ready ? (*p.ready)(k, first, cnt) : hipSuccess;
@@ -2179,8 +2200,7 @@
   const cg_signable_tmpl* dt = (const cg_signable_tmpl*)c->tmpls.p;
   if (d.fused) {
     if (d.n_tmpls) e = hipMemcpyAsync(c->tmpls.p, d.tmpls, sizeof(cg_signable_tmpl) * d.n_tmpls, hipMemcpyHostToDevice, s);
-    if (e == hipSuccess)
-      e = cg::launch_tx_sig_templates(dt, d.n_tmpls, d.arena, d.arena_len, slot, d.ids, d.n_ids, (uint8_t*)c->msgs.p, s);
+    if (e == hipSuccess) e = launch_templates(c, d.n_tmpls, d.arena, d.arena_len, slot, d.ids, d.n_ids, s);
   }
   const std::vector<uint64_t> bounds = cg::equal_bounds(d.n, chunk_of(c, d.n));
   for (size_t k = 0; e == hipSuccess && k + 1 < bounds.size(); ++k) {
@@ -2339,8 +2359,7 @@
   const cg_signable_tmpl* dt = (const cg_signable_tmpl*)c->tmpls.p;
   if (d.fused) {
     if (d.n_tmpls) e = hipMemcpyAsync(c->tmpls.p, d.tmpls, sizeof(cg_signable_tmpl) * d.n_tmpls, hipMemcpyHostToDevice, s);
-    if (e == hipSuccess)
-      e = cg::launch_tx_sig_templates(dt, d.n_tmpls, d.arena, d.arena_len, slot, d.ids, d.n_ids, (uint8_t*)c->msgs.p, s);
+    if (e == hipSuccess) e = launch_templates(c, d.n_tmpls, d.arena, d.arena_len, slot, d.ids, d.n_ids, s);
   }
   const std::vector<uint64_t> bounds = cg::equal_bounds(d.n, chunk_of(c, d.n));
   for (size_t k = 0; e == hipSuccess && k + 1 < bounds.size(); ++k) {
@@ -2519,8 +2538,7 @@
   const cg_signable_tmpl* dt = (const cg_signable_tmpl*)c->tmpls.p;
   if (d.fused) {
     if (d.n_tmpls) e = hipMemcpyAsync(c->tmpls.p, d.tmpls, sizeof(cg_signable_tmpl) * d.n_tmpls, hipMemcpyHostToDevice, s);
-    if (e == hipSuccess)
-      e = cg::launch_tx_sig_templates(dt, d.n_tmpls, d.arena, d.arena_len, slot, d.ids, d.n_ids, (uint8_t*)c->msgs.p, s);
+    if (e == hipSuccess) e = launch_templates(c, d.n_tmpls, d.arena, d.arena_len, slot, d.ids, d.n_ids, s);
   }
   const std::vector<uint64_t> bounds = cg::equal_bounds(d.n, chunk_of(c, d.n));
   for (size_t k = 0; e == hipSuccess && k + 1 < bounds.size(); ++k) {
diff --git a/corda_amd/csrc/engine.h b/corda_amd/csrc/engine.h
--- a/corda_amd/csrc/engine.h
+++ b/corda_amd/csrc/engine.h
@@ -322,7 +322,7 @@
                                uint8_t* d_msgs, hipStream_t stream);
 hipError_t launch_tx_sig_templates(const cg_signable_tmpl* d_tmpls, uint32_t n_tmpls, const uint8_t* d_arena,
                                    uint64_t arena_len, uint64_t slot, const uint8_t* d_ids, uint64_t n_ids,
-                                   uint8_t* d_msgs, hipStream_t stream);
+                                   uint8_t* d_msgs, hipStream_t stream, bool keep = false);
 hipError_t launch_tx_sig_range(const cg_txsig* d_sigs, uint64_t first, uint64_t n, const cg_signable_tmpl* d_tmpls,
                                uint32_t n_tmpls, const uint8_t* d_tx_status, uint64_t n_tx, const uint8_t* d_ids,
                                uint64_t arena_len, uint64_t slot, cg_item* d_items, uint8_t* d_msgs,
diff --git a/corda_amd/csrc/key_cache.h b/corda_amd/csrc/key_cache.h
--- a/corda_amd/csrc/key_cache.h
+++ b/corda_amd/csrc/key_cache.h
@@ -38,11 +38,26 @@
   const bool ok = len != 0 && len <= 4u * KC_KEY_WORDS && off <= arena_len && len <= arena_len - off;
   k.tag = ok ? (scheme & 0xffu) | (fmt & 0xffu) << 8 | len << 16 : 0u;
   const uint64_t lr = (arena_len + 3) & ~(uint64_t)3;
+  const uint64_t a0 = off & ~(uint64_t)3;
+  const uint32_t sh = (uint32_t)(off & 3) * 8u;
+  const uint32_t nw = ok ? ((uint32_t)(off & 3) + len + 3u) / 4u : 0u;
+  uint32_t aw[KC_KEY_WORDS + 1];
+#if defined(__HIP_DEVICE_COMPILE__)
+#pragma unroll
+#endif
+  for (uint32_t j = 0; j <= KC_KEY_WORDS; ++j) {
+    const bool in = j < nw && a0 + 4u * j < lr;
+    aw[j] = ok ? *(const uint32_t*)(arena + (in ? a0 + 4u * j : a0)) : 0u;
+    if (!in) aw[j] = 0u;
+  }
   uint32_t h = 0x811c9dc5u ^ k.tag;
+#if defined(__HIP_DEVICE_COMPILE__)
+#pragma unroll
+#endif
   for (uint32_t w = 0; w < KC_KEY_WORDS; ++w) {
     uint32_t v = 0;
     if (ok && 4u * w < len) {
-      v = kc_ld4(arena, lr, off + 4u * w);
+      v = sh == 0 ? aw[w] : (aw[w] >> sh) | (aw[w + 1] << (32u - sh));
       if (len - 4u * w < 4u) v &= (1u << (8u * (len - 4u * w))) - 1u;
     }
     k.bytes[w] = v;
@@ -69,10 +84,12 @@
   return hash & m & (size - 1u);
 }
 
+KC_HD uint32_t kc_begin_state(uint32_t state, bool dirty) { return !dirty && state == KC_VALID ? KC_VALID : KC_EMPTY; }
 KC_HD bool kc_begin_slot(KcOwner* owners, uint32_t* live, uint32_t s, bool dirty) {
-  if (dirty || owners[s].state != KC_VALID) owners[s].state = KC_EMPTY;
+  const uint32_t was = owners[s].state, now = kc_begin_state(was, dirty);
+  if (now != was) owners[s].state = now;
   live[s] = 0;
-  return owners[s].state == KC_VALID;
+  return now == KC_VALID;
 }
 
 KC_HD uint32_t kc_cas(uint32_t* p, uint32_t expect, uint32_t val) {
@@ -85,11 +102,14 @@
 #endif
 }
 
-KC_HD bool kc_index_insert(uint32_t* index, uint32_t size, uint32_t bits, const KcOwner* owners, uint32_t s) {
-  uint32_t b = kc_home(owners[s].key.hash, bits, size);
+KC_HD bool kc_index_insert_hash(uint32_t* index, uint32_t size, uint32_t bits, uint32_t hash, uint32_t s) {
+  uint32_t b = kc_home(hash, bits, size);
   for (uint32_t n = 0; n < size; ++n, b = (b + 1u) & (size - 1u))
     if (kc_cas(&index[b], 0u, s + 1u) == 0u) return true;
   return false;
+}
+KC_HD bool kc_index_insert(uint32_t* index, uint32_t size, uint32_t bits, const KcOwner* owners, uint32_t s) {
+  return kc_index_insert_hash(index, size, bits, owners[s].key.hash, s);
 }
 
 KC_HD uint32_t kc_probe(const uint32_t* index, uint32_t size, uint32_t bits, const KcOwner* owners, const KcKey& k) {
diff --git a/corda_amd/csrc/key_uses.h b/corda_amd/csrc/key_uses.h
--- /dev/null
+++ b/corda_amd/csrc/key_uses.h
@@ -0,0 +1,24 @@
+#pragma once
+#include <stdint.h>
+
+#if defined(__HIPCC__)
+#include <hip/hip_runtime.h>
+#endif
+#ifndef CG_HD
+#if defined(__HIPCC__)
+#define CG_HD __host__ __device__ __forceinline__
+#else
+#define CG_HD static inline
+#endif
+#endif
+
+#define KEY_USES_LDS_CAP 8192u
+#define KEY_USES_SAMPLE_UNIT 4u
+
+CG_HD bool key_uses_sampled(uint64_t i) { return (((uint32_t)i * 0x9E3779B1u) >> 30) == 0u; }
+
+CG_HD uint32_t key_uses_word(bool sampled) { return sampled ? 2u : 1u; }
+CG_HD uint32_t key_uses_apply(uint32_t h, bool sampled) { return sampled ? h + 2u : h | 1u; }
+
+CG_HD bool key_uses_seen(uint32_t h) { return h != 0u; }
+CG_HD uint32_t key_uses_add(uint32_t h) { return (h >> 1) * KEY_USES_SAMPLE_UNIT; }
diff --git a/corda_amd/csrc/sig12_scan.h b/corda_amd/csrc/sig12_scan.h
--- /dev/null
+++ b/corda_amd/csrc/sig12_scan.h
@@ -0,0 +1,47 @@
+#pragma once
+#include <stdint.h>
+
+#if defined(__HIPCC__)
+#include <hip/hip_runtime.h>
+#endif
+#ifndef CG_HD
+#if defined(__HIPCC__)
+#define CG_HD __host__ __device__ __forceinline__
+#else
+#define CG_HD static inline
+#endif
+#endif
+
+#define SIG12_SCAN_LANES 1024u
+#define SIG12_SCAN_PER 4u
+#define SIG12_SCAN_TILE (SIG12_SCAN_LANES * SIG12_SCAN_PER)
+
+CG_HD uint64_t sig12_scan_tiles(uint64_t nb) { return (nb + SIG12_SCAN_TILE - 1) / SIG12_SCAN_TILE; }
+
+CG_HD uint64_t sig12_scan_before(const uint64_t* raw, uint64_t end, uint32_t t) {
+  uint64_t s = 0;
+#if defined(__HIP_DEVICE_COMPILE__)
+#pragma unroll 8
+#endif
+  for (uint64_t i = t; i < end; i += SIG12_SCAN_LANES) s += raw[i];
+  return s;
+}
+
+CG_HD uint64_t sig12_scan_load(const uint64_t* raw, uint64_t nb, uint64_t tile, uint32_t t, uint64_t x[SIG12_SCAN_PER]) {
+  const uint64_t lo = tile * SIG12_SCAN_TILE + (uint64_t)t * SIG12_SCAN_PER;
+  uint64_t s = 0;
+  for (uint32_t q = 0; q < SIG12_SCAN_PER; ++q) {
+    x[q] = lo + q < nb ? raw[lo + q] : 0;
+    s += x[q];
+  }
+  return s;
+}
+
+CG_HD void sig12_scan_store(uint64_t* out, uint64_t nb, uint64_t tile, uint32_t t, const uint64_t x[SIG12_SCAN_PER],
+                            uint64_t run) {
+  const uint64_t lo = tile * SIG12_SCAN_TILE + (uint64_t)t * SIG12_SCAN_PER;
+  for (uint32_t q = 0; q < SIG12_SCAN_PER; ++q) {
+    if (lo + q < nb) out[lo + q] = run;
+    run += x[q];
+  }
+}
diff --git a/corda_amd/csrc/tmpl_keep.h b/corda_amd/csrc/tmpl_keep.h
--- /dev/null
+++ b/corda_amd/csrc/tmpl_keep.h
@@ -0,0 +1,52 @@
+#pragma once
+#include <stdint.h>
+
+#if defined(__HIPCC__)
+#include <hip/hip_runtime.h>
+#endif
+#ifndef CG_HD
+#if defined(__HIPCC__)
+#define CG_HD __host__ __device__ __forceinline__
+#else
+#define CG_HD static inline
+#endif
+#endif
+
+CG_HD uint32_t tmpl_ld4(const uint8_t* arena, uint64_t len_rounded, uint64_t off) {
+  const uint64_t a0 = off & ~(uint64_t)3;
+  const uint32_t sh = (uint32_t)(off & 3) * 8u;
+  const uint32_t w0 = a0 < len_rounded ? *(const uint32_t*)(arena + a0) : 0u;
+  if (sh == 0) return w0;
+  const uint32_t w1 = (a0 + 4) < len_rounded ? *(const uint32_t*)(arena + a0 + 4) : 0u;
+  return (w0 >> sh) | (w1 << (32u - sh));
+}
+
+CG_HD uint32_t tmpl_image_byte(bool ok, uint64_t prefix_off, uint32_t prefix_len, uint64_t suffix_off,
+                               uint32_t suffix_len, const uint8_t* arena, uint64_t len_rounded, uint64_t x) {
+  if (!ok) return 0u;
+  if (x < prefix_len) return tmpl_ld4(arena, len_rounded, prefix_off + x) & 0xffu;
+  if (x < (uint64_t)prefix_len + 32u) return 0u;
+  if (x < (uint64_t)prefix_len + 32u + suffix_len)
+    return tmpl_ld4(arena, len_rounded, suffix_off + (x - prefix_len - 32u)) & 0xffu;
+  return 0u;
+}
+
+CG_HD uint32_t tmpl_image_word(bool ok, uint64_t prefix_off, uint32_t prefix_len, uint64_t suffix_off,
+                               uint32_t suffix_len, const uint8_t* arena, uint64_t len_rounded, uint64_t x) {
+  if (!ok) return 0u;
+  const uint64_t id_end = (uint64_t)prefix_len + 32u, end = id_end + suffix_len;
+  if (x + 4 <= prefix_len) return tmpl_ld4(arena, len_rounded, prefix_off + x);
+  if (x >= prefix_len && x + 4 <= id_end) return 0u;
+  if (x >= id_end && x + 4 <= end) return tmpl_ld4(arena, len_rounded, suffix_off + (x - id_end));
+  if (x >= end) return 0u;
+  uint32_t v = 0;
+  for (uint32_t q = 0; q < 4; ++q)
+    v |= tmpl_image_byte(ok, prefix_off, prefix_len, suffix_off, suffix_len, arena, len_rounded, x + q) << (8 * q);
+  return v;
+}
+
+CG_HD bool tmpl_mid_kept(uint32_t kept_blocks, uint32_t kept_prefix_len, uint32_t kept_ed_mid, bool ok,
+                         uint32_t prefix_len, uint32_t ed_min) {
+  return kept_prefix_len == prefix_len && kept_blocks == (ok ? prefix_len / 64u : 0u) &&
+         kept_ed_mid == ((ok && prefix_len >= ed_min) ? 1u : 0u);
+}
diff --git a/corda_amd/csrc/txpipe.hip b/corda_amd/csrc/txpipe.hip
--- a/corda_amd/csrc/txpipe.hip
+++ b/corda_amd/csrc/txpipe.hip
@@ -3,6 +3,8 @@
 #include "engine.h"
 #include "keyws.h"
 #include "sha2.h"
+#include "sig12_scan.h"
+#include "tmpl_keep.h"
 
 namespace cg {
 
@@ -72,26 +74,30 @@
   }
 }
 
-__global__ void __launch_bounds__(1024) k_sig12_scan(uint64_t* __restrict__ sums, uint64_t nb, uint64_t base) {
-  __shared__ uint64_t sh[1024];
-  const uint32_t t = threadIdx.x;
-  const uint64_t per = (nb + 1023) / 1024, lo = t * per, hi = lo + per < nb ? lo + per : nb;
-  uint64_t s = 0;
-  for (uint64_t i = lo; i < hi; ++i) s += sums[i];
-  sh[t] = s;
+__global__ void __launch_bounds__(SIG12_SCAN_LANES) k_sig12_scan(const uint64_t* __restrict__ sums, uint64_t nb,
+                                                                 uint64_t base, uint64_t* __restrict__ bases) {
+  constexpr uint32_t W = SIG12_SCAN_LANES / 64;
+  __shared__ uint64_t w_before[W], w_own[W];
+  const uint32_t t = threadIdx.x, lane = t & 63u, wave = t >> 6;
+  const uint64_t tile = blockIdx.x;
+  uint64_t before = sig12_scan_before(sums, tile * SIG12_SCAN_TILE, t);
+  uint64_t x[SIG12_SCAN_PER];
+  const uint64_t own = sig12_scan_load(sums, nb, tile, t, x);
+  uint64_t incl = own;
+#pragma unroll
+  for (int d = 1; d < 64; d <<= 1) {
+    const uint64_t u = __shfl_up(incl, d, 64);
+    if ((int)lane >= d) incl += u;
+    before += __shfl_xor(before, d, 64);
+  }
+  if (lane == 63) {
+    w_own[wave] = incl;
+    w_before[wave] = before;
+  }
   __syncthreads();
-  for (uint32_t d = 1; d < 1024; d <<= 1) {
-    const uint64_t u = t >= d ? sh[t - d] : 0;
-    __syncthreads();
-    sh[t] += u;
-    __syncthreads();
-  }
-  uint64_t run = base + sh[t] - s;
-  for (uint64_t i = lo; i < hi; ++i) {
-    const uint64_t x = sums[i];
-    sums[i] = run;
-    run += x;
-  }
+  uint64_t run = base + incl - own;
+  for (uint32_t w = 0; w < W; ++w) run += w_before[w] + (w < wave ? w_own[w] : 0);
+  sig12_scan_store(bases, nb, tile, t, x, run);
 }
 
 __global__ void __launch_bounds__(SIG12_BLOCK) k_txsig12_items(const cg_txsig_packed* __restrict__ sigs, uint64_t first,
@@ -138,14 +144,16 @@
   items[first + jj] = it;
 }
 
-size_t tx_sig12_scratch_bytes(uint64_t n) { return 8 * ((n + SIG12_BLOCK - 1) / SIG12_BLOCK + 1); }
+size_t tx_sig12_scratch_bytes(uint64_t n) { return 16 * ((n + SIG12_BLOCK - 1) / SIG12_BLOCK + 1); }
 
 hipError_t launch_tx_sig12_bases(const cg_txsig_packed* d_sigs, uint64_t first, uint64_t n, uint64_t base,
                                  uint64_t* d_bases, hipStream_t stream) {
   if (n == 0) return hipSuccess;
   const uint64_t nb = (n + SIG12_BLOCK - 1) / SIG12_BLOCK;
-  hipLaunchKernelGGL(k_sig12_blocksum, dim3((unsigned)nb), dim3(SIG12_BLOCK), 0, stream, d_sigs, first, n, d_bases);
-  hipLaunchKernelGGL(k_sig12_scan, dim3(1), dim3(1024), 0, stream, d_bases, nb, base);
+  uint64_t* d_sums = d_bases + nb + 1;
+  hipLaunchKernelGGL(k_sig12_blocksum, dim3((unsigned)nb), dim3(SIG12_BLOCK), 0, stream, d_sigs, first, n, d_sums);
+  hipLaunchKernelGGL(k_sig12_scan, dim3((unsigned)sig12_scan_tiles(nb)), dim3(SIG12_SCAN_LANES), 0, stream,
+                     (const uint64_t*)d_sums, nb, base, d_bases);
   return hipGetLastError();
 }
 
@@ -175,7 +183,7 @@
 __global__ void __launch_bounds__(64) k_tmpl_prep(const cg_signable_tmpl* __restrict__ tmpls, uint32_t n_tmpls,
                                                   const uint8_t* __restrict__ arena, uint64_t arena_len,
                                                   uint64_t slot, const uint8_t* __restrict__ ids, uint64_t n_ids,
-                                                  uint8_t* __restrict__ msgs) {
+                                                  uint32_t keep, uint8_t* __restrict__ msgs) {
   const uint32_t t = blockIdx.x;
   if (t == 0 && threadIdx.x == 0) {
     SpliceHdr h;
@@ -191,19 +199,21 @@
   const bool ok = tmpl_ok(tm, arena_len);
   const uint64_t lr = round4(arena_len);
   auto byte_at = [&](uint64_t x) -> uint32_t {
-    if (!ok) return 0u;
-    if (x < tm.prefix_len) return cg_ld_bytes4(arena, lr, tm.prefix_off + x) & 0xffu;
-    if (x < tm.prefix_len + 32u) return 0u;
-    if (x < (uint64_t)tm.prefix_len + 32u + tm.suffix_len)
-      return cg_ld_bytes4(arena, lr, tm.suffix_off + (x - tm.prefix_len - 32u)) & 0xffu;
-    return 0u;
+    return tmpl_image_byte(ok, tm.prefix_off, tm.prefix_len, tm.suffix_off, tm.suffix_len, arena, lr, x);
+  };
+  auto word_at = [&](uint32_t w) -> uint32_t {
+    return tmpl_image_word(ok, tm.prefix_off, tm.prefix_len, tm.suffix_off, tm.suffix_len, arena, lr, 4ull * w);
   };
   uint32_t* img = (uint32_t*)(msgs + tx_img_off(n_tmpls) + (uint64_t)t * slot);
-  for (uint32_t w = threadIdx.x; w < slot / 4; w += 64) {
-    uint32_t v = 0;
-    for (int q = 0; q < 4; ++q) v |= byte_at(4ull * w + q) << (8 * q);
-    img[w] = v;
-  }
+  TmplMid* mid = (TmplMid*)(msgs + SPLICE_HDR_BYTES) + t;
+  if (keep) {
+    bool same = true;
+    for (uint32_t w = threadIdx.x; w < slot / 4; w += 64) same = same && img[w] == word_at(w);
+    if (threadIdx.x == 0)
+      same = same && tmpl_mid_kept(mid->blocks, mid->prefix_len, mid->ed_mid, ok, tm.prefix_len, TMPL_ED_MID_MIN_PREFIX);
+    if (__all(same)) return;
+  }
+  for (uint32_t w = threadIdx.x; w < slot / 4; w += 64) img[w] = word_at(w);
   const bool ed_mid = ok && tm.prefix_len >= TMPL_ED_MID_MIN_PREFIX;
   if (threadIdx.x == 1) {
     uint64_t* wk = ((TmplW512*)(msgs + tmpl_w512_off(n_tmpls)) + t)->wk;
@@ -236,14 +246,14 @@
       r.blocks = b + 1;
     }
   }
-  ((TmplMid*)(msgs + SPLICE_HDR_BYTES))[t] = r;
+  *mid = r;
 }
 
 hipError_t launch_tx_sig_templates(const cg_signable_tmpl* d_tmpls, uint32_t n_tmpls, const uint8_t* d_arena,
                                    uint64_t arena_len, uint64_t slot, const uint8_t* d_ids, uint64_t n_ids,
-                                   uint8_t* d_msgs, hipStream_t stream) {
+                                   uint8_t* d_msgs, hipStream_t stream, bool keep) {
   hipLaunchKernelGGL(k_tmpl_prep, dim3(n_tmpls ? n_tmpls : 1), dim3(64), 0, stream, d_tmpls, n_tmpls, d_arena,
-                     arena_len, slot, d_ids, n_ids, d_msgs);
+                     arena_len, slot, d_ids, n_ids, keep ? 1u : 0u, d_msgs);
   return hipGetLastError();
 }
 
diff --git a/corda_amd/csrc/verify.hip b/corda_amd/csrc/verify.hip
--- a/corda_amd/csrc/verify.hip
+++ b/corda_amd/csrc/verify.hip
@@ -1,3 +1,4 @@
+#include "key_uses.h"
 #include "keyws.h"
 
 namespace cg {
@@ -31,27 +32,58 @@
   wide_idx[i] = KEY_NOT_WIDE;
 }
 
-__global__ void __launch_bounds__(256) k_key_uses(const cg_item* __restrict__ items, uint64_t n_items,
-                                                  uint32_t n_keys, uint32_t* __restrict__ uses,
-                                                  uint8_t* __restrict__ seen) {
+template <class Rec>
+__global__ void __launch_bounds__(256) k_key_uses_global(const Rec* __restrict__ recs, uint64_t n, uint32_t n_keys,
+                                                         uint32_t* __restrict__ uses, uint8_t* __restrict__ seen) {
   const uint64_t i = (uint64_t)blockIdx.x * blockDim.x + threadIdx.x;
-  if (i >= n_items) return;
-  const uint32_t k = items[i].key_idx;
+  if (i >= n) return;
+  const uint32_t k = recs[i].key_idx;
   if (k >= n_keys) return;
   seen[k] = 1;
-  if (((uint32_t)i * 0x9E3779B1u) >> 30 == 0) atomicAdd(&uses[k], KEY_USES_SAMPLE);
-}
-
-template <class Sig>
-__global__ void __launch_bounds__(256) k_key_uses_txsig(const Sig* __restrict__ sigs, uint64_t n,
-                                                        uint32_t n_keys, uint32_t* __restrict__ uses,
-                                                        uint8_t* __restrict__ seen) {
-  const uint64_t i = (uint64_t)blockIdx.x * blockDim.x + threadIdx.x;
-  if (i >= n) return;
-  const uint32_t k = sigs[i].key_idx;
-  if (k >= n_keys) return;
-  seen[k] = 1;
-  if (((uint32_t)i * 0x9E3779B1u) >> 30 == 0) atomicAdd(&uses[k], KEY_USES_SAMPLE);
+  if (key_uses_sampled(i)) atomicAdd(&uses[k], KEY_USES_SAMPLE);
+}
+
+#define KEY_USES_BLOCK 1024
+#define KEY_USES_GRID 512u
+template <class Rec>
+__global__ void __launch_bounds__(KEY_USES_BLOCK) k_key_uses_lds(const Rec* __restrict__ recs, uint64_t n,
+                                                                 uint32_t n_keys, uint32_t* __restrict__ uses,
+                                                                 uint8_t* __restrict__ seen) {
+  __shared__ uint32_t hist[KEY_USES_LDS_CAP];
+  for (uint32_t k = threadIdx.x; k < n_keys; k += KEY_USES_BLOCK) hist[k] = 0;
+  __syncthreads();
+  const uint64_t step = (uint64_t)gridDim.x * KEY_USES_BLOCK;
+  for (uint64_t i0 = (uint64_t)blockIdx.x * KEY_USES_BLOCK + threadIdx.x; i0 < n; i0 += 4 * step) {
+    uint32_t k[4];
+#pragma unroll
+    for (int q = 0; q < 4; ++q) k[q] = i0 + q * step < n ? recs[i0 + q * step].key_idx : 0xffffffffu;
+#pragma unroll
+    for (int q = 0; q < 4; ++q) {
+      if (k[q] >= n_keys) continue;
+      if (key_uses_sampled(i0 + q * step)) atomicAdd(&hist[k[q]], key_uses_word(true));
+      else atomicOr(&hist[k[q]], key_uses_word(false));
+    }
+  }
+  __syncthreads();
+  for (uint32_t k = threadIdx.x; k < n_keys; k += KEY_USES_BLOCK) {
+    const uint32_t h = hist[k];
+    if (!key_uses_seen(h)) continue;
+    seen[k] = 1;
+    if (key_uses_add(h)) atomicAdd(&uses[k], key_uses_add(h));
+  }
+}
+static_assert(KEY_USES_SAMPLE == KEY_USES_SAMPLE_UNIT, "key_uses.h mirrors keyws.h");
+
+template <class Rec>
+static void launch_key_uses(const Rec* recs, uint64_t n, uint32_t n_keys, uint32_t* uses, uint8_t* seen,
+                            bool force_global, hipStream_t s) {
+  const uint64_t nb = (n + KEY_USES_BLOCK - 1) / KEY_USES_BLOCK;
+  const unsigned grid = (unsigned)(nb < KEY_USES_GRID ? nb : KEY_USES_GRID);
+  if (!force_global && n_keys <= KEY_USES_LDS_CAP)
+    hipLaunchKernelGGL(k_key_uses_lds<Rec>, dim3(grid), dim3(KEY_USES_BLOCK), 0, s, recs, n, n_keys, uses, seen);
+  else
+    hipLaunchKernelGGL(k_key_uses_global<Rec>, dim3((unsigned)((n + 255) / 256)), dim3(256), 0, s, recs, n, n_keys,
+                       uses, seen);
 }
 
 __global__ void __launch_bounds__(256) k_key_counts(const uint32_t* __restrict__ counts, uint32_t n_keys,
@@ -84,11 +116,33 @@
   uint32_t* index = kc.index[pool];
   if (threadIdx.x < KC_CTRS) kc.ctr[pool * KC_CTRS + threadIdx.x] = 0;
   for (uint32_t b = threadIdx.x; b < kc.size; b += KC_BLOCK) index[b] = 0;
-  for (uint32_t s = threadIdx.x; s < kc.slots; s += KC_BLOCK) kc_begin_slot(owners, kc.live[pool], s, kc.dirty);
+  constexpr uint32_t PER = KEY_WIDE_MAX / KC_BLOCK;
+  uint32_t st[PER], hs[PER];
+#pragma unroll
+  for (uint32_t j = 0; j < PER; ++j) {
+    const uint32_t s = threadIdx.x + j * KC_BLOCK;
+    st[j] = s < kc.slots ? owners[s].state : (uint32_t)KC_EMPTY;
+    hs[j] = s < kc.slots ? owners[s].key.hash : 0u;
+  }
+#pragma unroll
+  for (uint32_t j = 0; j < PER; ++j) {
+    const uint32_t s = threadIdx.x + j * KC_BLOCK;
+    if (s >= kc.slots) continue;
+    const uint32_t now = kc_begin_state(st[j], kc.dirty);
+    if (now != st[j]) owners[s].state = now;
+    st[j] = now;
+    kc.live[pool][s] = 0;
+  }
+  for (uint32_t s = threadIdx.x + PER * KC_BLOCK; s < kc.slots; s += KC_BLOCK)
+    kc_begin_slot(owners, kc.live[pool], s, kc.dirty);
   __syncthreads();
-  for (uint32_t s = threadIdx.x; s < kc.slots; s += KC_BLOCK)
+#pragma unroll
+  for (uint32_t j = 0; j < PER; ++j)
+    if (st[j] == KC_VALID) kc_index_insert_hash(index, kc.size, kc.bits, hs[j], threadIdx.x + j * KC_BLOCK);
+  for (uint32_t s = threadIdx.x + PER * KC_BLOCK; s < kc.slots; s += KC_BLOCK)
     if (owners[s].state == KC_VALID) kc_index_insert(index, kc.size, kc.bits, owners, s);
 }
+static_assert(KEY_WIDE_MAX % KC_BLOCK == 0, "k_kc_begin's lanes take KEY_WIDE_MAX / KC_BLOCK slots each");
 
 __device__ __forceinline__ void kc_load_key(KcKey& k, const cg_key& key, const uint8_t* arena, uint64_t arena_len) {
   kc_key_load(k, key.scheme, key.fmt, key.len, arena, arena_len, key.off);
@@ -113,40 +167,57 @@
     else if (u == 0) u = 1;
     uses[i] = u;
   }
+  int pool = -1;
   if (i < n_keys && u >= ED_DIRECT_MAX_USES) {
     const uint8_t s = keys[i].scheme;
     c = s == CG_EDDSA_ED25519_SHA512 ? PLAN_ED
       : s == CG_ECDSA_SECP256R1_SHA256 ? PLAN_R1
       : s == CG_ECDSA_SECP256K1_SHA256 ? PLAN_K1
                                        : -1;
-    const int pool = c == PLAN_ED ? 0 : 1;
-    if (c >= 0 && u >= (pool == 0 ? min_ed : min_ec) && u != KEY_USES_ALL) {
-      const uint32_t cap = pool == 0 ? cap_ed : cap_ec;
-      if (cap) {
-        const uint32_t slot = atomicAdd(&wide_count[PLAN_CLASSES + pool], 1u);
-        if (slot < cap) {
-          is_wide = true;
-          if (!kc.on()) {
-            wide_idx[i] = slot;
-            cw = c;
-          } else {
-            KcKey k;
-            kc_load_key(k, keys[i], arena, arena_len);
-            const uint32_t hit = kc_probe(kc.index[pool], kc.size, kc.bits, kc.owners[pool], k);
-            if (hit != KC_NONE) {
-              wide_idx[i] = hit;
-              kc.live[pool][hit] = 1;
-              atomicAdd(&kc.ctr[pool * KC_CTRS + KC_CTR_HITS], 1u);
-            } else {
-              cw = c;
-            }
-          }
-          c = -1;
-        } else if (kc.on()) {
-          atomicAdd(&kc.ctr[pool * KC_CTRS + KC_CTR_FELL_BACK], 1u);
+    const int p = c == PLAN_ED ? 0 : 1;
+    if (c >= 0 && u >= (p == 0 ? min_ed : min_ec) && u != KEY_USES_ALL && (p == 0 ? cap_ed : cap_ec)) pool = p;
+  }
+  const uint32_t lane = threadIdx.x & 63u;
+  uint32_t slot = 0xffffffffu;
+  for (int p = 0; p < 2; ++p) {
+    const uint64_t m = __ballot(pool == p);
+    if (m == 0) continue;
+    const int leader = __ffsll((long long)m) - 1;
+    uint32_t base = 0;
+    if ((int)lane == leader) base = atomicAdd(&wide_count[PLAN_CLASSES + p], (uint32_t)__popcll(m));
+    base = __shfl(base, leader, 64);
+    if (pool == p) slot = base + (uint32_t)__popcll(m & ((1ull << lane) - 1ull));
+  }
+  bool hit_slot = false, fell_back = false;
+  if (pool >= 0) {
+    if (slot < (pool == 0 ? cap_ed : cap_ec)) {
+      is_wide = true;
+      if (!kc.on()) {
+        wide_idx[i] = slot;
+        cw = c;
+      } else {
+        KcKey k;
+        kc_load_key(k, keys[i], arena, arena_len);
+        const uint32_t hit = kc_probe(kc.index[pool], kc.size, kc.bits, kc.owners[pool], k);
+        if (hit != KC_NONE) {
+          wide_idx[i] = hit;
+          kc.live[pool][hit] = 1;
+          hit_slot = true;
+        } else {
+          cw = c;
         }
       }
+      c = -1;
+    } else if (kc.on()) {
+      fell_back = true;
     }
+  }
+  for (int p = 0; p < 2; ++p) {
+    const uint64_t mh = __ballot(pool == p && hit_slot), mf = __ballot(pool == p && fell_back);
+    if (mh && (int)lane == __ffsll((long long)mh) - 1)
+      atomicAdd(&kc.ctr[p * KC_CTRS + KC_CTR_HITS], (uint32_t)__popcll(mh));
+    if (mf && (int)lane == __ffsll((long long)mf) - 1)
+      atomicAdd(&kc.ctr[p * KC_CTRS + KC_CTR_FELL_BACK], (uint32_t)__popcll(mf));
   }
   if (i < n_keys && u >= 1 && !is_wide) {
     const uint8_t s = keys[i].scheme;
@@ -318,6 +389,7 @@
   const KeyUses* src;
   KeyWs w;
   uint32_t all;
+  bool uses_global = false;
 };
 
 struct HipOps {
@@ -365,8 +437,7 @@
         return kOk;
       }
       case cgs::ST_KEY_USES:
-        hipLaunchKernelGGL(k_key_uses, dim3((unsigned)((key->n_items + 255) / 256)), dim3(256), 0, s, key->d_items,
-                           key->n_items, key->r.n_keys, key->w.uses, key->w.seen);
+        launch_key_uses(key->d_items, key->n_items, key->r.n_keys, key->w.uses, key->w.seen, key->uses_global, s);
         return kOk;
       case cgs::ST_KEY_COUNTS:
         hipLaunchKernelGGL(k_key_counts, dim3((key->r.n_keys + 255) / 256), dim3(256), 0, s, key->src->counts,
@@ -374,9 +445,7 @@
         return kOk;
       case cgs::ST_KEY_USES_TXSIG:
         with_records(key->src->sigs, [&](auto* recs) {
-          using Rec = std::remove_const_t<std::remove_pointer_t<decltype(recs)>>;
-          hipLaunchKernelGGL(k_key_uses_txsig<Rec>, dim3((unsigned)((key->src->n + 255) / 256)), dim3(256), 0, s, recs,
-                             key->src->n, key->r.n_keys, key->w.uses, key->w.seen);
+          launch_key_uses(recs, key->src->n, key->r.n_keys, key->w.uses, key->w.seen, key->uses_global, s);
         });
         return kOk;
       case cgs::ST_KC_BEGIN:
@@ -504,7 +573,7 @@
   const cg_item* d_items = src ? nullptr : r.d_items;
   const uint64_t n_items = src ? src->n : r.n_items;
   const bool counted = d_items || src;
-  const KeyArgs key = {r, d_items, n_items, src, key_ws(d_keyprep, n_keys, counted ? wide : nullptr), counted ? 0u : 1u};
+  KeyArgs key = {r, d_items, n_items, src, key_ws(d_keyprep, n_keys, counted ? wide : nullptr), counted ? 0u : 1u};
   cgs::KeyPlan k;
   k.any_keys = n_keys != 0;
   k.counted = counted;
@@ -519,6 +588,8 @@
   }();
   for (int f = 0; f < 3; ++f)
     if ((test_skip >> f) & 1u) k.need_full[f] = false;
+  const char* ug = getenv("CG_TEST_KEY_USES_GLOBAL");
+  key.uses_global = ug && ug[0] == '1';
   k.cache = key.w.kc.on();
   k.wide_ed = key.w.cap_ed != 0;
   k.wide_ec = key.w.cap_ec != 0;
```

After: 456.6 million (median of 4 runs). About the same (+1.7%).
